# andrei-ace/EdgeStyle

Hardware: AMD Instinct MI355X
Metric: 512x512 try-on images/sec @ 50 DDIM steps (6-cond ControlNet) (higher is better)
Workload: dtype f16; 1 GPU; BASELINE configs[1]: full 6-cond edgestyle_multicontrolnet + controllora, 512x512, 50 DDIM steps, CFG 7.5, batch=1/GPU, hipGraph-captured step, cond embedding + VAE decode included; images_per_gpu=1, ddim_steps=50, parallelism=dp1 (independent images, one RCCL gather)

## Files before the change

### edgestyle_amd/csrc/builder.hip

```cpp
#include <hip/hip_runtime.h>
#include <math.h>
#include <stdio.h>
#include <stdlib.h>
#include <string.h>

#include <algorithm>
#include <deque>
#include <functional>
#include <map>
#include <memory>
#include <stdexcept>
#include <string>
#include <thread>
#include <unordered_map>
#include <vector>

#include "../../include/edgestyle_hip.h"
#include "plan.h"

extern "C" void es_set_error(const char* msg);
extern "C" int es_plan_set_dry(int on);

namespace {

// ... 335 lines not shown
bool groups_tile_256(const es_launch_query& q) {
  for (int g = 0; g < std::min(q.n_counts, 4); ++g) if ((q.group_n[g] * q.hw) % 256) return false;
  return true;
}
bool launch_takes_xs(const es_launch_query& q, const es_launch_knobs& k) {
  const bool xs_res = !q.has_residual || (k.xs_residual && q.kpad == 320 && !q.geglu && !q.has_ln && q.residual_dense && !(q.wide && wide_stream(q.dtype, k)));
  if (!(q.ksize == 1 && q.stride == 1 && !q.upsample && !q.C2 && !q.has_temb && xs_res && !q.n_tails && q.x_rep == 1 && q.act == ES_ACT_NONE &&
        q.unit_scale && !q.force_splitk && !k.force_bn && k.xs_enabled)) return false;
  if (q.ngroups > 1 && (q.ngroups > 4 || !groups_tile_256(q) || !q.groups_agree)) return false;
  return xs_shape_ok(q.M, q.ksize, q.kpad, q.cin, q.ctail, q.cout, q.geglu != 0, k.xs_min_m);
}
bool launch_choose(const es_launch_query& q, const es_launch_knobs& k, es_launch_choice* o) {
  memset(o, 0, sizeof(*o));
  if (launch_takes_xs(q, k)) { o->route = ES_ROUTE_LINEAR_XS; return true; }
  const bool aligned = q.C1 % BK == 0 && q.C2 % BK == 0;
  const bool big_ok = k.big_tile && aligned && !q.geglu && !q.has_ln && groups_tile_256(q);
  const bool small_ok = k.small_tile && aligned && !q.geglu && k.force_waves != 8;
  const bool ln256_ok = k.big_tile_256 && (q.geglu || q.has_ln) && q.ksize == 1 && q.stride == 1 && !q.upsample && !q.C2 && !q.n_tails && !q.has_temb &&
                        q.x_rep == 1 && q.C1 % BK == 0 && q.rows_padded % 256 == 0 && q.cout % 8 == 0 && !(q.geglu && q.has_residual) && !q.wide &&
                        q.gn_groups == 0 && k.force_waves != 8 && groups_tile_256(q);
  int cand[5], nc = 0;
  if (ln256_ok) cand[nc++] = 256;
  if (big_ok) cand[nc++] = 320;
  cand[nc++] = 160; cand[nc++] = 128;
  if (small_ok) cand[nc++] = 64;
  if (k.force_bn) { cand[0] = k.force_bn; nc = 1; }
  const bool geglu = q.geglu != 0, allow_split = !q.has_ln;
  int bn, splitk, stages;
  if (!plan_gemm(q.M, q.rows_padded, q.kpad, geglu, cand, nc, allow_split, &bn, &splitk, &stages)) return false;
  if (bn == 320 && !k.force_bn && (q.force_splitk ? q.force_splitk : splitk) == 1 &&
      !es_conv_gemm8p_form_ok(geglu ? ES_ACT_GEGLU : q.act, q.cout, q.has_temb, q.hw, q.has_residual)) {
    const int at = (int)(std::find(cand, cand + nc, 320) - cand);
    std::copy(cand + at + 1, cand + nc, cand + at);
    if (!plan_gemm(q.M, q.rows_padded, q.kpad, geglu, cand, nc - 1, allow_split, &bn, &splitk, &stages)) return false;
  }
  if (stages == 4 && !k.deep_ring) stages = 2;
  if (q.force_splitk) { splitk = q.force_splitk; stages = q.stages; }
  else if (q.stages) stages = q.stages;
  if (!stages) stages = k.force_stages;
  o->bn = bn; o->splitk = splitk; o->stages = stages;
  if (k.force_waves) o->waves = k.force_waves;
  else if (k.eight_waves && q.ksize == 1 && q.M <= 65536 && aligned && bn != 64 && bn != 320 && bn != 256 && !(stages == 4 && bn != 128) && stages != 3) o->waves = 8;
  o->xcd_m_fastest = k.xcd_order < 0 ? (q.ngroups <= 1 && splitk == 1 && q.M <= 2048 && q.w_numel > q.src_numel) : k.xcd_order;
  const int cstore = geglu ? q.cout / 2 : q.cout;
  o->gn_partials = q.gn_groups > 0 && gn_handover(q.hw, cstore, q.gn_groups, k) && !geglu && !q.has_ln && q.cout / q.gn_groups <= (bn == 320 ? 160 : bn);
  o->wide = q.wide && q.has_residual && wide_stream(q.dtype, k) && cstore % 8 == 0 && !geglu;
  return true;
}
bool launch_gn_fold(const es_launch_query& q, int groups, const es_launch_knobs& k) {
  if (!(k.gn_fold && k.xs_enabled) || k.gn_handover || q.hw % 256 || groups < 1 || groups > 32) return false;
  if (q.geglu || q.has_ln || q.kpad % groups || !xs_shape_fits(q.ksize, q.kpad, q.cin, q.ctail, q.cout, false)) return false;
  if (q.M < (q.kpad == 320 ? 8192 : 32768)) return false;
  return !(q.ngroups > 1 && (q.ngroups > 4 || !groups_tile_256(q) || !q.groups_agree));
}
struct BuildEnv { es_launch_knobs knobs; bool chunk_major; };
BuildEnv read_build_env() {
  auto env = [](const char* name, const char* dflt) { const char* e = getenv(name); return std::string(e ? e : dflt); };
  const std::string ho = env("ES_GN_HANDOVER", "0"), ws = env("ES_WIDE_STREAM", "auto");
  BuildEnv b;
  b.chunk_major = env("ES_CHUNK_MAJOR", "0") == "1";
  es_launch_knobs& k = b.knobs;
  memset(&k, 0, sizeof(k));
  k.xs_enabled = k.big_tile = k.small_tile = k.eight_waves = k.deep_ring = 1; k.xs_min_m = XS_MIN_M; k.xcd_order = -1;
  k.xs_residual = env("ES_XS_RESIDUAL", "1") == "1"; k.big_tile_256 = env("ES_BIG_TILE_256", "1")[0] != '0'; k.gn_fold = env("ES_GN_FOLD", "1") == "1";
  k.gn_handover = ho == "all" ? 2 : ho == "1"; k.wide_stream = ws == "auto" ? -1 : ws == "1";
  return b;
}

struct Builder {
  Heap heap;
  unsigned long long ws_bytes = 0;
  int dt = ES_F16;
  const BuildEnv env = read_build_env();
  std::vector<std::pair<unsigned long long, std::vector<char>>> uploads;
  std::deque<PW> pws;
  std::map<std::string, const PW*> pack_cache;
  std::map<const void*, unsigned long long> vec_cache;
  std::map<std::pair<int, int>, unsigned long long> gn_partials, fusion_scratch;
  std::map<int, unsigned long long> zero_bias;

  T empty(int n, int h, int w, int c, int es = 2) {
    T t; t.n = n; t.h = h; t.w = w; t.c = c; t.ld = c; t.es = es;
    auto blk = std::make_shared<Blk>();
    blk->heap = &heap; blk->bytes = std::max<size_t>(t.bytes(), 1); blk->off = heap.alloc(blk->bytes);
    t.b = blk; t.p = FAKE_HEAP + blk->off;
    return t;
  }
  unsigned long long persistent(size_t bytes) { return FAKE_HEAP + heap.alloc(std::max<size_t>(bytes, 1)); }
  T persistent_t(int n, int h, int w, int c, int es = 2) {
    T t; t.n = n; t.h = h; t.w = w; t.c = c; t.ld = c; t.es = es;
    t.p = persistent(t.bytes());
    return t;
  }
  char* staged(unsigned long long addr, size_t bytes) {
    uploads.emplace_back(addr, std::vector<char>(bytes, 0));
    return uploads.back().second.data();
  }
  unsigned long long upload_f32(const std::vector<float>& v) {
    const unsigned long long a = persistent(v.size() * 4);
    memcpy(staged(a, v.size() * 4), v.data(), v.size() * 4);
    return a;
  }
  unsigned long long workspace(unsigned long long bytes) { ws_bytes = std::max(ws_bytes, bytes); return FAKE_WS; }
  void add_into(const T& a, const T& b, const T& out) {
    if (!a.contig() || !b.contig() || !out.contig() || a.numel() != b.numel() || a.numel() != out.numel()) fail("builder: add of non-contiguous or differently sized tensors");
    ok(es_add(a.ptr(), b.ptr(), out.ptr(), a.numel(), dt, nullptr), "es_add");
// ... 313 lines not shown
    return out;
  }

  T group_norm(const T& x, const std::vector<Norm>& nl, int groups, float eps, bool silu, const T& x2 = T(), const std::vector<int>& group_n = {}) {
    const int N = x.n, C1 = x.c, C2 = x2 ? x2.c : 0;
    T out = empty(N, x.h, x.w, C1 + C2);
    auto key = std::make_pair(N, groups);
    auto it = gn_partials.find(key);
    if (it == gn_partials.end()) it = gn_partials.emplace(key, persistent(es_group_norm_partials_bytes(N, groups))).first;
    es_gn_desc d;
    memset(&d, 0, sizeof(d));
    d.x = x.ptr(); d.x2 = x2 ? x2.ptr() : nullptr; d.out = out.ptr(); d.partials = (float*)it->second;
    if (nl.size() > 1) {
      int sum = 0;
      for (int n : group_n) sum += n;
      if (nl.size() > 4 || group_n.size() != nl.size() || sum != N) fail("grouped group_norm: bad group table");
      d.ngroups = (int)nl.size();
      int acc = 0;
      for (size_t g = 0; g < nl.size(); ++g) { acc += group_n[g]; d.n_end[g] = acc; d.gamma_g[g] = (const float*)nl[g].g; d.beta_g[g] = (const float*)nl[g].b; }
    } else { d.gamma = (const float*)nl[0].g; d.beta = (const float*)nl[0].b; }
    d.N = N; d.HW = (int)x.hw(); d.C1 = C1; d.C2 = C2; d.groups = groups; d.eps = eps; d.silu = silu; d.dtype = dt;
    if (x.gnp && !x2 && gn_handover(x.hw(), C1, groups, env.knobs) && x.gnp_groups == groups) {
      d.partials = (float*)x.gnp; d.ext_chunks = (int)(2 * (x.hw() / 64));
    }
    ok(es_group_norm(&d, nullptr), "es_group_norm");
    return out;
  }
  T group_norm(const T& x, const Norm& n, int groups, float eps, bool silu, const T& x2 = T()) { return group_norm(x, std::vector<Norm>{n}, groups, eps, silu, x2); }

  T gn_proj_in(const T& x, const std::vector<Norm>& nl, int groups, float eps, const PWs& pl, const std::vector<int>& group_n = {}) {
    const int N = x.n;
    const long long hw = x.hw(), M = (long long)N * hw;
    const bool grouped = pl.size() > 1;
    CA g; g.group_n = group_n;
    es_launch_query q = launch_query(pl, M, hw, g, x.c, 0, x.numel(), false);
    for (const PW* p : pl)
      if (p->rows_padded != pl[0]->rows_padded || p->kpad != pl[0]->kpad || p->cout != pl[0]->cout || p->geglu != pl[0]->geglu) q.groups_agree = 0;
    if (!(x.contig() && launch_gn_fold(q, groups, env.knobs))) return conv_gemm(group_norm(x, nl, groups, eps, false, T(), group_n), pl, g);
    auto key = std::make_pair(N, groups);
    auto it = gn_partials.find(key);
    if (it == gn_partials.end()) it = gn_partials.emplace(key, persistent(es_group_norm_partials_bytes(N, groups))).first;
    es_gn_desc d;
    memset(&d, 0, sizeof(d));
    d.x = x.ptr(); d.partials = (float*)it->second;
    d.N = N; d.HW = (int)hw; d.C1 = x.c; d.C2 = 0; d.groups = groups; d.eps = eps; d.silu = 0; d.dtype = dt; d.stats_only = 1;
    ok(es_group_norm(&d, nullptr), "es_group_norm");
    T out = empty(N, x.h, x.w, pl[0]->cout);
    GnFront gn;
    gn.part = it->second; gn.nl = nl; gn.groups = groups; gn.nchunk = es_group_norm_chunks((int)hw); gn.hw = (int)hw; gn.eps = eps;
    std::vector<long long> rows;
    if (grouped) for (int n : group_n) rows.push_back(n * hw);
    linear_xs(x.view((int)M, 1, 1, x.c), pl, M, out.view((int)M, 1, 1, pl[0]->cout), rows, T(), &gn);
    return out;
  }

  T timestep_embedding(const T& t, int n, int dim) {
    T out = empty(n, 1, 1, dim);
    ok(es_timestep_embedding((const float*)t.ptr(), out.ptr(), n, dim, dt, nullptr), "es_timestep_embedding");
    return out;
  }
  void memcpy_t(const T& dst, const T& src) {
    if (!dst.contig() || !src.contig() || dst.bytes() != src.bytes()) fail("memcpy: contiguous tensors of equal byte size");
    ok(es_memcpy(dst.ptr(), src.ptr(), src.bytes(), nullptr), "es_memcpy");
  }
  void memcpy2d(unsigned long long dst, size_t dpitch, unsigned long long src, size_t spitch, size_t width, size_t height) {
    ok(es_memcpy2d((void*)dst, dpitch, (const void*)src, spitch, width, height, nullptr), "es_memcpy2d");
  }
  void gather_row(const T& table, int nrows, const T& idx, const T& out, int row_len) {
    ok(es_gather_row((const float*)table.ptr(), (const int32_t*)idx.ptr(), (float*)out.ptr(), row_len, nrows, nullptr), "es_gather_row");
  }
};

struct UCfg {
  int in_ch, out_ch, nb, ch[4], has_attn[4], lpb, heads, cross, groups; float eps;
  int nce, ce[4], cond_ch;
};
struct VCfg { int nb, ch[4], lpb, latent, groups; float eps, scaling; int scale() const { return 1 << (nb - 1); } };

struct Resnet {
  Norm n1, n2;
  const PW *conv1 = nullptr, *conv2 = nullptr, *shortc = nullptr, *conv2s = nullptr;
  int groups = 32; float eps = 1e-5f; int temb_off = -1;
  Resnet() {}
  Resnet(Builder& B, const Weights& W, const std::string& p, int groups_, float eps_, int temb_off_) : groups(groups_), eps(eps_), temb_off(temb_off_) {
    const es_tensor* w1 = W.get(p + ".conv1.weight");
    const int cin = (int)w1->shape[1], cout = (int)w1->shape[0];
    W.shaped(p + ".conv1.weight", {cout, cin, 3, 3}); W.shaped(p + ".conv2.weight", {cout, cout, 3, 3});
    if (W.has(p + ".conv_shortcut.weight")) W.shaped(p + ".conv_shortcut.weight", {cout, cin, 1, 1});
    else if (cin != cout) fail("es_load_weights: '" + p + "' changes the channel count but has no conv_shortcut");
    if (temb_off_ >= 0) W.shaped(p + ".time_emb_proj.weight", {cout, -1});
    n1 = B.norm(W, p + ".norm1", cin); n2 = B.norm(W, p + ".norm2", cout);
    conv1 = B.conv(W, p + ".conv1");
    const bool has_short = W.has(p + ".conv_shortcut.weight");
    if (has_short && cout % 64 == 0 && cin % 64 == 0) conv2s = B.conv_tail(W, p + ".conv2", p + ".conv_shortcut");
    else { conv2 = B.conv(W, p + ".conv2"); if (has_short) shortc = B.conv(W, p + ".conv_shortcut"); }
  }
  T run(Builder& B, const T& x, const T& tproj, const T& x2 = T()) const {
    T h = B.group_norm(x, n1, groups, eps, true, x2);
    CA a;
    if (temb_off >= 0) { a.temb = tproj.chan(temb_off, tproj.c - temb_off); a.temb_stride = tproj.ld; }
    a.gn_groups = groups;
    h = B.conv_gemm(h, conv1, a);
    h = B.group_norm(h, n2, groups, eps, true);
    if (conv2s) {
      if (x2 && (x.c % 64 || x2.c % 64)) fail("builder: skip concat with channels that are not multiples of 64");
      CA t; t.tails.push_back(x); if (x2) t.tails.push_back(x2); t.gn_groups = groups;
// ... 249 lines not shown
    }
    h = B.group_norm(h, d_norm, cfg.groups, cfg.eps, true);
    return B.conv_gemm(h, d_out);
  }
};

struct Model {
  Builder B;
  UCfg ucfg; VCfg vcfg;
  es_ctx_geometry geo;
  Dict d_unet, d_vae, d_fusion, d_cn[6];
  UNet unet;
  VAE vae;
  std::vector<std::unique_ptr<ControlNet>> nets;
  std::vector<int> net_of_cond;
  std::vector<std::pair<int, std::vector<int>>> groups;
  std::vector<FusionParams> fusion;
  std::vector<std::pair<int, int>> table;
  std::vector<const Encoder*> encs; std::vector<int> counts; int ntot = 0, width = 0, ncn = 0;
  int B_ = 1, N = 2, T_ = 50, h = 64, w = 64, nn = 6, kmax = 3;
  T latents, model_in, noise, ehs, step_idx, t_rows, scales_cur, t_table, scale_table, coef, ts_dev, image;
  std::vector<T> conds, cond_img, cond_noise, gbufs, hist;
  std::vector<T> ctx_grouped, ctx_unet; std::vector<std::vector<T>> ctx_nets;
  T cond_cat, tproj_table, tproj_cur, tproj_gen;
  std::vector<T> fused_zero, fz_zero, fz_u;
  bool guess = false;
  int Bc = 2;
  std::vector<std::vector<T>> ctx_guess;

  std::vector<Norm> norms(const std::vector<const Resnet*>& rs, int which) const { std::vector<Norm> v; for (auto r : rs) v.push_back(which == 1 ? r->n1 : r->n2); return v; }

  T g_resnet(const std::vector<const Resnet*>& rs, const T& x, const T& tproj) {
    const Resnet* r0 = rs[0];
    T hh = B.group_norm(x, norms(rs, 1), r0->groups, r0->eps, true, T(), counts);
    PWs c1, c2, c2s, sh; bool all_s = true;
    for (auto r : rs) { c1.push_back(r->conv1); c2.push_back(r->conv2); c2s.push_back(r->conv2s); sh.push_back(r->shortc); if (!r->conv2s) all_s = false; }
    CA a; a.temb = tproj.chan(r0->temb_off, tproj.c - r0->temb_off); a.temb_stride = tproj.ld; a.group_n = counts; a.gn_groups = r0->groups;
    hh = B.conv_gemm(hh, c1, a);
    hh = B.group_norm(hh, norms(rs, 2), r0->groups, r0->eps, true, T(), counts);
    if (all_s) { CA t; t.tails.push_back(x); t.group_n = counts; t.gn_groups = r0->groups; return B.conv_gemm(hh, c2s, t); }
    for (auto r : rs) if (r->conv2s) fail("builder: grouped resnets must fold conv_shortcut all alike");
    T xs = x;
    if (r0->shortc) { CA s; s.group_n = counts; xs = B.conv_gemm(x, sh, s); }
    CA r; r.residual = xs; r.group_n = counts; r.wide = true; r.gn_groups = r0->groups;
    return B.conv_gemm(hh, c2, r);
  }
  T g_transformer(const std::vector<const Transformer*>& ts, const T& x, const T& kv) {
    const Transformer* t0 = ts[0];
    const int Nn = x.n, H = x.h, Wd = x.w, C = x.c;
    std::vector<int> rows;
    for (int n : counts) rows.push_back(n * H * Wd);
    std::vector<Norm> nl; PWs pin, qkv, o1, q2, o2, ff1, ffo;
    for (auto t : ts) { nl.push_back(t->norm); pin.push_back(t->proj_in); qkv.push_back(t->qkv_ln); o1.push_back(t->o1); q2.push_back(t->q2_ln); o2.push_back(t->o2); ff1.push_back(t->ff1_ln); ffo.push_back(t->ffo); }
    T tok = B.gn_proj_in(x, nl, t0->groups, 1e-6f, pin, counts).view(Nn, H * Wd, 1, C);
    CA gr; gr.group_n = rows;
    T q = B.linear(tok, qkv, gr);
    T a = B.attention(q.chan(0, C), q.chan(C, C), q.chan(2 * C, C), t0->heads);
    CA r1 = gr; r1.residual = tok; r1.wide = true;
    tok = B.linear(a, o1, r1);
    T qq = B.linear(tok, q2, gr);
    a = B.attention(qq, kv.chan(0, C), kv.chan(C, C), t0->heads);
    CA r2 = gr; r2.residual = tok; r2.wide = true;
    tok = B.linear(a, o2, r2);
    T f = B.linear(tok, ff1, gr);
    CA fo; fo.x2 = tok.view(Nn, H, Wd, C); fo.residual = x; fo.group_n = counts; fo.wide = true; fo.gn_groups = t0->groups;
    return B.conv_gemm(f.view(Nn, H, Wd, 4 * C), ffo, fo);
  }
  void g_run(T hh, const T& tproj, std::vector<T>& skips, T& mid) {
    const Encoder* e0 = encs[0];
    skips.push_back(hh);
    int ci = 0;
    auto rs_of = [&](const std::function<const Resnet*(const Encoder*)>& f) { std::vector<const Resnet*> v; for (auto e : encs) v.push_back(f(e)); return v; };
    auto ts_of = [&](int ti) { std::vector<const Transformer*> v; for (auto e : encs) v.push_back(&e->tr[ti]); return v; };
    for (size_t i = 0; i < e0->down.size(); ++i) {
      for (size_t j = 0; j < e0->down[i].size(); ++j) {
        hh = g_resnet(rs_of([&](const Encoder* e) { return &e->down[i][j].first; }), hh, tproj);
        if (e0->down[i][j].second >= 0) { hh = g_transformer(ts_of(e0->down[i][j].second), hh, ctx_grouped[ci]); ++ci; }
        skips.push_back(hh);
      }
      if (e0->downsample[i]) {
        PWs ds; for (auto e : encs) ds.push_back(e->downsample[i]);
        CA a; a.stride = 2; a.group_n = counts; a.gn_groups = ucfg.groups;
        hh = B.conv_gemm(hh, ds, a);
        skips.push_back(hh);
      }
    }
    hh = g_resnet(rs_of([](const Encoder* e) { return &e->mid0; }), hh, tproj);
    hh = g_transformer(ts_of(e0->mid_attn), hh, ctx_grouped[ci]);
    mid = g_resnet(rs_of([](const Encoder* e) { return &e->mid1; }), hh, tproj);
  }
  T transformer(const Transformer& t, const T& x, const T& kv) {
    const int Nn = x.n, H = x.h, Wd = x.w, C = x.c;
    T tok = B.gn_proj_in(x, std::vector<Norm>{t.norm}, t.groups, 1e-6f, PWs{t.proj_in}).view(Nn, H * Wd, 1, C);
    T q = B.linear(tok, t.qkv_ln);
    T a = B.attention(q.chan(0, C), q.chan(C, C), q.chan(2 * C, C), t.heads);
    CA r1; r1.residual = tok; r1.wide = true;
    tok = B.linear(a, t.o1, r1);
    T qq = B.linear(tok, t.q2_ln);
    a = B.attention(qq, kv.chan(0, C), kv.chan(C, C), t.heads);
    CA r2; r2.residual = tok; r2.wide = true;
    tok = B.linear(a, t.o2, r2);
    T f = B.linear(tok, t.ff1_ln);
    CA fo; fo.x2 = tok.view(Nn, H, Wd, C); fo.residual = x; fo.wide = true; fo.gn_groups = t.groups;
    return B.conv_gemm(f.view(Nn, H, Wd, 4 * C), t.ffo, fo);
  }

  void set_context() {
    size_t gi = 0;
    for (const auto& g : groups) {
      const ControlNet& net = *nets[g.first];
      for (int ti = 0; ti < net.n_enc_tr; ++ti) net.tr[ti].context(B, ehs, ctx_nets[gi][ti], (int)g.second.size());
      ++gi;
    }
    for (size_t ti = 0; ti < unet.tr.size(); ++ti) unet.tr[ti].context(B, ehs, ctx_unet[ti], 1);
  }
  void set_conds() {
    int a = 0;
    for (const auto& g : groups) for (int p : g.second) { B.memcpy_t(cond_cat.batch(a, N), conds[p]); a += N; }
  }
  void set_time_table() {
    int a = 0;
    const size_t es = 2;
    for (size_t e = 0; e < encs.size(); ++e) {
      T proj = encs[e]->time_proj(B, ts_dev, T_);
      const size_t wb = (size_t)encs[e]->tproj_width() * es;
      for (int j = 0; j < counts[e]; ++j)
        B.memcpy2d(tproj_table.p + (unsigned long long)(a + j) * width * es, (size_t)ntot * width * es, proj.p, wb, wb, (size_t)T_);
      a += counts[e];
    }
  }
  T time_proj_generic() {
    const size_t es = 2;
    int a = 0;
    for (size_t e = 0; e < encs.size(); ++e) {
      T proj = encs[e]->time_proj(B, t_rows, counts[e]);
      const size_t wb = (size_t)encs[e]->tproj_width() * es;
      B.memcpy2d(tproj_gen.p + (unsigned long long)a * width * es, (size_t)width * es, proj.p, wb, wb, (size_t)counts[e]);
      a += counts[e];
    }
    return tproj_gen;
  }
  std::vector<T> fuse(const std::vector<std::vector<T>>& rpn, int Nf, const std::vector<T>* addends) {
    const size_t nl = rpn[0].size();
    std::vector<es_fusion_desc> fd(nl);
    std::vector<T> us, outs;
    for (size_t k = 0; k < nl; ++k) {
      const FusionParams& fp = fusion[k];
      const int HW = fp.s * fp.s, Cc = fp.c;
      auto key = std::make_pair(Nf, (int)k);
      auto it = B.fusion_scratch.find(key);
      if (it == B.fusion_scratch.end()) it = B.fusion_scratch.emplace(key, B.persistent(es_fusion_scratch_bytes(Nf))).first;
      T u = B.empty(Nf, HW, 1, Cc), out = B.empty(Nf, HW, 1, Cc);
      es_fusion_desc& d = fd[k];
      memset(&d, 0, sizeof(d));
      for (int i = 0; i < 6; ++i) { d.res[i] = rpn[i][k].ptr(); d.res_bs[i] = rpn[i][k].bstride(); d.res_scale[i] = 1.f; }
// ... 202 lines not shown
      }
    }
  }

  void pack_fusion(const Weights& W) {
    for (size_t i = 0; i < table.size(); ++i) {
      const std::string p = i + 1 < table.size() ? "multi_controlnet_down_blocks." + std::to_string(i) : "multi_controlnet_mid_block";
      const int c = table[i].first, s = table[i].second, hw = s * s;
      FusionParams f; f.c = c; f.s = s;
      f.w1 = B.upload_f32(to_f32(W.shaped(p + ".first_conv.weight", {3 * c, 2, 1, 1})));
      f.b1 = B.upload_f32(to_f32(W.shaped(p + ".first_conv.bias", {3 * c})));
      f.w2 = B.upload_f32(to_f32(W.shaped(p + ".second_conv.weight", {c, 3, 1, 1})));
      f.b2 = B.upload_f32(to_f32(W.shaped(p + ".second_conv.bias", {c})));
      f.w3 = B.upload_f32(to_f32(W.shaped(p + ".third_conv.weight", {c, 1, 1, 1})));
      f.b3 = B.upload_f32(to_f32(W.shaped(p + ".third_conv.bias", {c})));
      auto plane = [&](const std::string& key, int per) {
        const std::vector<float> t = to_f32(W.shaped(key, {(long long)per * c, s, s}));
        const unsigned long long a = B.persistent((size_t)hw * c * per * 2);
        uint16_t* d = (uint16_t*)B.staged(a, (size_t)hw * c * per * 2);
        parallel_for(hw, [&](long long x0, long long x1) {
          for (long long px = x0; px < x1; ++px)
            for (int cc = 0; cc < c * per; ++cc) d[(size_t)px * c * per + cc] = B.enc(t[(size_t)cc * hw + px]);
        });
        return a;
      };
      f.g1 = plane(p + ".first_normalization.weight", 3); f.be1 = plane(p + ".first_normalization.bias", 3);
      f.g2 = plane(p + ".second_normalization.weight", 1); f.be2 = plane(p + ".second_normalization.bias", 1);
      fusion.push_back(f);
    }
  }
};

struct Recording {
  es_plan* p;
  explicit Recording(es_plan* pl) : p(pl) { if (es_plan_begin_record(p)) fail(std::string("es_load_weights: ") + es_last_error()); es_plan_set_dry(1); }
  ~Recording() { es_plan_set_dry(0); es_plan_end_record(p); }
};

}

extern "C" int es_plan_gemm_choice(long long M, int rows_padded, int kpad, int geglu, const int* bns, int n_bns, int allow_split, int* bn, int* splitk, int* stages) {
  if (!bns || n_bns < 1 || !bn || !splitk || !stages) { es_set_error("es_plan_gemm_choice: null argument"); return -1; }
  if (!plan_gemm(M, rows_padded, kpad, geglu != 0, bns, n_bns, allow_split != 0, bn, splitk, stages)) { es_set_error("es_plan_gemm_choice: rows_padded fits no N tile"); return -1; }
  return 0;
}
extern "C" int es_linear_xs_eligible(long long M, int ksize, int kpad, int cin, int ctail, int cout, int geglu) {
  return xs_shape_ok(M, ksize, kpad, cin, ctail, cout, geglu != 0, XS_MIN_M) ? 1 : 0;
}
extern "C" int es_launch_choose(const es_launch_query* q, const es_launch_knobs* k, es_launch_choice* out) {
  if (!q || !k || !out) { es_set_error("es_launch_choose: null argument"); return -1; }
  if (!launch_choose(*q, *k, out)) { es_set_error("es_launch_choose: rows_padded fits no N tile"); return -1; }
  return 0;
}
extern "C" int es_launch_route(const es_launch_query* q, const es_launch_knobs* k) { return q && k && launch_takes_xs(*q, *k) ? ES_ROUTE_LINEAR_XS : ES_ROUTE_CONV_GEMM; }
extern "C" int es_launch_gn_fold(const es_launch_query* q, int groups, const es_launch_knobs* k) { return q && k && launch_gn_fold(*q, groups, *k); }
extern "C" int es_launch_gn_handover(long long hw, int c, int groups, const es_launch_knobs* k) { return k && gn_handover(hw, c, groups, *k); }
extern "C" int es_launch_wide_stream(int dtype, const es_launch_knobs* k) { return k && wide_stream(dtype, *k); }

extern "C" int es_load_weights(const es_weights* wts, const es_model_config* mc, const es_ctx_geometry* g, int device, es_ctx** out) {
  if (!wts || !mc || !g || !out) { es_set_error("es_load_weights: null argument"); return -1; }
  es_ctx* ctx = nullptr;
  es_plan* plans[ES_PLAN_COUNT] = {};
  void* arena = nullptr;
  try {
    auto m = std::make_unique<Model>();
    Model& M = *m;
    Builder& B = M.B;
    if (mc->n_blocks < 2 || mc->n_blocks > 4 || mc->vae_n_blocks < 2 || mc->vae_n_blocks > 4) fail("es_load_weights: 2..4 resolution levels");
    if (g->n_conds != 6 && g->n_conds != 1) fail("es_load_weights: n_conds is 6 (the reference's fused multi-ControlNet model, MC:66-114) or 1 (a single ControlNet, PL:338-351)");
    if (g->n_conds == 1 && wts->n_controlnets != 1) fail("es_load_weights: a single-ControlNet context takes exactly one ControlNet");
    if (g->dtype != ES_F16 && g->dtype != ES_BF16) fail("es_load_weights: dtype must be ES_F16 or ES_BF16");
    if (g->B < 1 || g->h < 1 || g->w < 1 || g->n_steps < 1) fail("es_load_weights: bad geometry");
    if (wts->n_controlnets < 1 || wts->n_controlnets > 6) fail("es_load_weights: 1..6 distinct ControlNets");
    UCfg& u = M.ucfg;
    u.in_ch = mc->in_channels; u.out_ch = mc->out_channels; u.nb = mc->n_blocks; u.lpb = mc->layers_per_block; u.heads = mc->num_heads;
    u.cross = mc->cross_attention_dim; u.groups = mc->norm_num_groups; u.eps = mc->norm_eps; u.nce = mc->n_cond_embed; u.cond_ch = mc->conditioning_channels;
    for (int i = 0; i < 4; ++i) { u.ch[i] = mc->block_out_channels[i]; u.has_attn[i] = mc->down_has_attn[i]; u.ce[i] = mc->cond_embed_channels[i]; }
    VCfg& v = M.vcfg;
    v.nb = mc->vae_n_blocks; v.lpb = mc->vae_layers_per_block; v.latent = mc->vae_latent_channels; v.groups = mc->vae_norm_num_groups;
    v.eps = mc->vae_norm_eps; v.scaling = mc->vae_scaling_factor;
    for (int i = 0; i < 4; ++i) v.ch[i] = mc->vae_block_out_channels[i];
    if (u.in_ch != v.latent) fail("es_load_weights: the UNet's in_channels must equal the VAE's latent_channels");
    if (u.cond_ch != 3 || u.nce < 2 || u.nce > 4) fail("es_load_weights: conditioning embedding of 3 input channels, 2..4 widths");
    M.geo = *g;
    B.dt = g->dtype;
    M.B_ = g->B; M.N = g->cfg ? 2 * g->B : g->B; M.T_ = g->n_steps; M.h = g->h; M.w = g->w; M.nn = g->n_conds;
    M.guess = g->guess_mode != 0;
    M.Bc = M.guess ? g->B : M.N;
    const int N = M.N, TS = M.T_, h = g->h, w = g->w, Bn = g->B, NN = g->n_conds, Nc = M.Bc;
    if (!M.guess) {
      int cnt[6] = {};
      for (int p = 0; p < NN; ++p) {
        const int ni = wts->net_of_cond[p];
        if (ni < 0 || ni >= wts->n_controlnets) fail("es_load_weights: net_of_cond names a ControlNet that was not given");
        ++cnt[ni];
      }
      const int hw_min = (h >> (u.nb - 1)) * (w >> (u.nb - 1));
      for (int i = 0; i <= wts->n_controlnets; ++i) {
        const long long n = (i < wts->n_controlnets ? (long long)cnt[i] : 1) * N;
        if (n && (n * hw_min) % BM) fail("es_load_weights: the groups of the lockstep pass do not tile in 128-pixel units at this latent size (the Python host falls back to serial chains; this builder does not)");
      }
    }
    M.d_unet.init(wts->unet, "UNet"); M.d_vae.init(wts->vae, "VAE"); M.d_fusion.init(wts->fusion, "fusion");
    for (int i = 0; i < wts->n_controlnets; ++i) M.d_cn[i].init(wts->controlnet[i], ("ControlNet " + std::to_string(i)).c_str());
    Weights Wu; Wu.own = &M.d_unet; Wu.who = "UNet";
    Weights Wv; Wv.own = &M.d_vae; Wv.who = "VAE";
// ... 202 lines not shown
```

### edgestyle_amd/csrc/elementwise.hip

```cpp
#include "common.h"
#include "../../include/edgestyle_hip.h"
#include "plan.h"
#include <string.h>

namespace {

thread_local char g_err[256] = "";

template <typename T>
__global__ void timestep_kernel(const float* __restrict__ t, T* __restrict__ out, int N, int dim) {
  const int half = dim / 2;
  const int i = blockIdx.x * blockDim.x + threadIdx.x;
  if (i >= N * half) return;
  const int n = i / half, k = i - n * half;
  const float f = expf(-9.210340371976184f * (float)k / (float)half);
  const float a = t[n] * f;
  out[(size_t)n * dim + k] = from_f32<T>(cosf(a));
  out[(size_t)n * dim + half + k] = from_f32<T>(sinf(a));
}

template <typename T>
__global__ void cfg_ddim_kernel(const T* __restrict__ noise, float* __restrict__ lat, T* __restrict__ model_in,
                                const float* __restrict__ coef, const int* __restrict__ step_idx, float gs, int B,
                                int HW, int L, int Ls, int cfg, int nsteps) {
// ... 282 lines not shown
  if (es_plan_recording()) { const es_op_incr a{ctr}; es_plan_record(ES_OP_INCR, &a, sizeof(a)); ES_PLAN_DRY_RETURN(); }
  hipLaunchKernelGGL(incr_kernel, dim3(1), dim3(1), 0, (hipStream_t)stream, ctr);
  ES_RET("es_incr");
}

extern "C" int es_gather_row(const float* table, const int32_t* idx, float* out, int row_len, int nrows,
                             void* stream) {
  if (!table || !idx || !out || row_len < 1 || nrows < 1) { es_set_error("es_gather_row: bad arguments"); return -1; }
  if (es_plan_recording()) { const es_op_gather_row a{table, idx, out, row_len, nrows}; es_plan_record(ES_OP_GATHER_ROW, &a, sizeof(a)); ES_PLAN_DRY_RETURN(); }
  hipLaunchKernelGGL(gather_row_kernel, dim3(nblk(row_len)), dim3(256), 0, (hipStream_t)stream, table, idx, out,
                     row_len, nrows);
  ES_RET("es_gather_row");
}

extern "C" int es_latents_to_input(const float* latents, void* model_in, int B, int HW, int L, int Lstride, int cfg,
                                   int dtype, void* stream) {
  if (!latents || !model_in || B < 1 || HW < 1 || L < 1 || Lstride < L) { es_set_error("es_latents_to_input: bad arguments"); return -1; }
  if (es_plan_recording()) { const es_op_latents_to_input a{latents, model_in, B, HW, L, Lstride, cfg, dtype}; es_plan_record(ES_OP_LATENTS_TO_INPUT, &a, sizeof(a)); ES_PLAN_DRY_RETURN(); }
  const long long n = (long long)B * HW * Lstride;
  if (dtype == ES_F16) hipLaunchKernelGGL(latents_to_input_kernel<f16>, dim3(nblk(n)), dim3(256), 0, (hipStream_t)stream, latents, (f16*)model_in, B, HW, L, Lstride, cfg);
  else hipLaunchKernelGGL(latents_to_input_kernel<bf16>, dim3(nblk(n)), dim3(256), 0, (hipStream_t)stream, latents, (bf16*)model_in, B, HW, L, Lstride, cfg);
  ES_RET("es_latents_to_input");
}

extern "C" int es_memcpy(void* dst, const void* src, size_t bytes, void* stream) {
  if (!dst || !src || !bytes) { es_set_error("es_memcpy: bad arguments"); return -1; }
  if (es_plan_recording()) { const es_op_memcpy a{dst, src, bytes}; es_plan_record(ES_OP_MEMCPY, &a, sizeof(a)); ES_PLAN_DRY_RETURN(); }
  if (hipMemcpyAsync(dst, src, bytes, hipMemcpyDeviceToDevice, (hipStream_t)stream) != hipSuccess) { es_set_error("es_memcpy: hipMemcpyAsync failed"); return -2; }
  return 0;
}

extern "C" int es_memcpy2d(void* dst, size_t dpitch, const void* src, size_t spitch, size_t width, size_t height, void* stream) {
  if (!dst || !src || !width || !height || dpitch < width || spitch < width) { es_set_error("es_memcpy2d: bad arguments"); return -1; }
  if (es_plan_recording()) { const es_op_memcpy2d a{dst, dpitch, src, spitch, width, height}; es_plan_record(ES_OP_MEMCPY2D, &a, sizeof(a)); ES_PLAN_DRY_RETURN(); }
  if (hipMemcpy2DAsync(dst, dpitch, src, spitch, width, height, hipMemcpyDeviceToDevice, (hipStream_t)stream) != hipSuccess) { es_set_error("es_memcpy2d: hipMemcpy2DAsync failed"); return -2; }
  return 0;
}

extern "C" int es_fill_f32(float* dst, float value, size_t n, void* stream) {
  if (!dst || !n) { es_set_error("es_fill_f32: bad arguments"); return -1; }
  if (es_plan_recording()) { const es_op_fill_f32 a{dst, n, value}; es_plan_record(ES_OP_FILL_F32, &a, sizeof(a)); ES_PLAN_DRY_RETURN(); }
  if (hipMemsetD32Async((hipDeviceptr_t)dst, __builtin_bit_cast(int, value), n, (hipStream_t)stream) != hipSuccess) { es_set_error("es_fill_f32: hipMemsetD32Async failed"); return -2; }
  return 0;
}

extern "C" size_t es_sizeof_desc(int which) {
  switch (which) {
    case 0: return sizeof(es_gemm_desc);
    case 1: return sizeof(es_attn_desc);
    case 2: return sizeof(es_gn_desc);
    case 3: return sizeof(es_fusion_desc);
    case 4: return sizeof(es_ln_desc);
    case 5: return sizeof(es_xs_desc);
    default: return 0;
  }
}
```

### edgestyle_amd/csrc/plan.h

```cpp
#pragma once
#include <stddef.h>
#include <stdint.h>

enum es_op_kind {
  ES_OP_CONV_GEMM = 1, ES_OP_LINEAR_XS, ES_OP_ATTENTION, ES_OP_GROUP_NORM, ES_OP_LAYER_NORM, ES_OP_LAYER_NORM_GROUPED,
  ES_OP_FUSION_BLOCK, ES_OP_FUSION_BLOCKS, ES_OP_TIMESTEP_EMBEDDING, ES_OP_CFG_DDIM, ES_OP_CFG_UNIPC, ES_OP_NCHW_TO_NHWC,
  ES_OP_NHWC_TO_NCHW, ES_OP_ADD, ES_OP_VAE_SAMPLE, ES_OP_INCR, ES_OP_GATHER_ROW, ES_OP_MEMCPY, ES_OP_MEMCPY2D,
  ES_OP_FILL_F32, ES_OP_LATENTS_TO_INPUT,
};

struct es_op_layer_norm { const void* x; void* out; const float* gamma; const float* beta; int M, C; float eps; int dtype; };
struct es_op_timestep { const float* t; void* out; int N, dim, dtype, pad_; };
struct es_op_cfg_ddim { const void* noise; float* latents; void* model_in; const float* coef; const int32_t* step_idx;
                        float guidance_scale; int B, HW, L, Lstride, cfg, nsteps, dtype; };
struct es_op_cfg_unipc { const void* noise; float* latents; float* last_sample; float* m0; float* m1; void* model_in;
                         const float* coef; const int32_t* step_idx; float guidance_scale; int B, HW, L, Lstride, cfg, nsteps, dtype; };
struct es_op_nchw_to_nhwc { const float* in; void* out; int N, C, HW, Cpad, dtype, pad_; };
struct es_op_nhwc_to_nchw { const void* in; float* out; int N, C, HW, Cstride; float scale, shift; int clamp01, dtype; };
struct es_op_add { const void* a; const void* b; void* y; int64_t n; int dtype, pad_; };
struct es_op_vae_sample { const void* moments; const float* noise; void* z; int N, HW, L, Lpad; float scaling; int dtype; };
struct es_op_incr { int32_t* ctr; };
struct es_op_gather_row { const float* table; const int32_t* idx; float* out; int row_len, nrows; };
struct es_op_memcpy { void* dst; const void* src; size_t bytes; };
struct es_op_memcpy2d { void* dst; size_t dpitch; const void* src; size_t spitch; size_t width, height; };
struct es_op_fill_f32 { float* dst; size_t n; float value; int pad_; };
struct es_op_latents_to_input { const float* latents; void* model_in; int B, HW, L, Lstride, cfg, dtype; };

extern "C" int es_plan_recording(void);
extern "C" void es_plan_record(int kind, const void* args, size_t bytes);
extern "C" int es_plan_dry(void);
#define ES_PLAN_RECORD(kind, ptr, bytes) do { if (es_plan_recording()) { es_plan_record((kind), (ptr), (bytes)); if (es_plan_dry()) return 0; } } while (0)
#define ES_PLAN_DRY_RETURN() do { if (es_plan_dry()) return 0; } while (0)

struct es_plan;
struct es_ctx;
int es_plan_relocate(es_plan* p, unsigned long long (*map)(unsigned long long addr, int use, void* user), void* user);
void es_ctx_adopt_arena(es_ctx* c, void* arena, size_t bytes, bool on_host);
void es_ctx_add_extent(es_ctx* c, unsigned long long off, unsigned long long bytes);

int es_image_resize_impl(const char* who, const es_image_u8* imgs, int count, uint8_t* out_u8, float* const* out_f32,
                         const int32_t* normalize, int R, void* workspace, size_t workspace_bytes, void* stream);

int es_randn_impl(const char* who, float* out, const es_randn_desc* d, void* stream, unsigned long long* advance);
```

### edgestyle_amd/csrc/plan.hip

```cpp
#include <hip/hip_runtime.h>
#include <dlfcn.h>
#include <math.h>
#include <stdio.h>
#include <stdlib.h>
#include <string.h>
#include <algorithm>
#include <string>
#include <utility>
#include <vector>

#include "../../include/edgestyle_hip.h"
#include "plan.h"

extern "C" void es_set_error(const char* msg);

struct es_plan {
  struct Op { int kind; size_t off, bytes; };
  std::vector<Op> ops;
  std::vector<char> blob;
};

namespace {
thread_local es_plan* g_rec = nullptr;
thread_local bool g_replaying = false;
thread_local bool g_dry = false;

struct RunOpts { const float* guidance = nullptr; const es_ctx* unipc = nullptr; };
int unipc_step(const es_ctx* c, const es_op_cfg_ddim* r, float guidance, void* s);

int launch_op(const es_plan* p, const es_plan::Op& op, hipStream_t st, const RunOpts& ro) {
  const float* guidance_override = ro.guidance;
  const char* a = p->blob.data() + op.off;
  void* s = (void*)st;
  switch (op.kind) {
    case ES_OP_CONV_GEMM: return es_conv_gemm((const es_gemm_desc*)a, s);
    case ES_OP_LINEAR_XS: return es_linear_xs((const es_xs_desc*)a, s);
    case ES_OP_ATTENTION: return es_attention((const es_attn_desc*)a, s);
    case ES_OP_GROUP_NORM: return es_group_norm((const es_gn_desc*)a, s);
    case ES_OP_LAYER_NORM: { auto* r = (const es_op_layer_norm*)a; return es_layer_norm(r->x, r->out, r->gamma, r->beta, r->M, r->C, r->eps, r->dtype, s); }
    case ES_OP_LAYER_NORM_GROUPED: return es_layer_norm_grouped((const es_ln_desc*)a, s);
    case ES_OP_FUSION_BLOCK: return es_fusion_block((const es_fusion_desc*)a, s);
    case ES_OP_FUSION_BLOCKS: return es_fusion_blocks((const es_fusion_desc*)a, (int)(op.bytes / sizeof(es_fusion_desc)), s);
    case ES_OP_TIMESTEP_EMBEDDING: { auto* r = (const es_op_timestep*)a; return es_timestep_embedding(r->t, r->out, r->N, r->dim, r->dtype, s); }
    case ES_OP_CFG_DDIM: { auto* r = (const es_op_cfg_ddim*)a;
      if (ro.unipc) return unipc_step(ro.unipc, r, guidance_override ? *guidance_override : r->guidance_scale, s);
      return es_cfg_ddim_step(r->noise, r->latents, r->model_in, r->coef, r->step_idx, guidance_override ? *guidance_override : r->guidance_scale,
                              r->B, r->HW, r->L, r->Lstride, r->cfg, r->nsteps, r->dtype, s); }
    case ES_OP_CFG_UNIPC: { auto* r = (const es_op_cfg_unipc*)a;
      return es_cfg_unipc_step(r->noise, r->latents, r->last_sample, r->m0, r->m1, r->model_in, r->coef, r->step_idx,
                               guidance_override ? *guidance_override : r->guidance_scale, r->B, r->HW, r->L, r->Lstride, r->cfg, r->nsteps, r->dtype, s); }
    case ES_OP_NCHW_TO_NHWC: { auto* r = (const es_op_nchw_to_nhwc*)a; return es_nchw_f32_to_nhwc(r->in, r->out, r->N, r->C, r->HW, r->Cpad, r->dtype, s); }
    case ES_OP_NHWC_TO_NCHW: { auto* r = (const es_op_nhwc_to_nchw*)a; return es_nhwc_to_nchw_f32(r->in, r->out, r->N, r->C, r->HW, r->Cstride, r->scale, r->shift, r->clamp01, r->dtype, s); }
    case ES_OP_ADD: { auto* r = (const es_op_add*)a; return es_add(r->a, r->b, r->y, r->n, r->dtype, s); }
    case ES_OP_VAE_SAMPLE: { auto* r = (const es_op_vae_sample*)a; return es_vae_sample(r->moments, r->noise, r->z, r->N, r->HW, r->L, r->Lpad, r->scaling, r->dtype, s); }
    case ES_OP_INCR: { auto* r = (const es_op_incr*)a; return es_incr(r->ctr, s); }
    case ES_OP_GATHER_ROW: { auto* r = (const es_op_gather_row*)a; return es_gather_row(r->table, r->idx, r->out, r->row_len, r->nrows, s); }
    case ES_OP_MEMCPY: { auto* r = (const es_op_memcpy*)a; return es_memcpy(r->dst, r->src, r->bytes, s); }
    case ES_OP_MEMCPY2D: { auto* r = (const es_op_memcpy2d*)a; return es_memcpy2d(r->dst, r->dpitch, r->src, r->spitch, r->width, r->height, s); }
    case ES_OP_FILL_F32: { auto* r = (const es_op_fill_f32*)a; return es_fill_f32(r->dst, r->value, r->n, s); }
    case ES_OP_LATENTS_TO_INPUT: { auto* r = (const es_op_latents_to_input*)a; return es_latents_to_input(r->latents, r->model_in, r->B, r->HW, r->L, r->Lstride, r->cfg, r->dtype, s); }
    default: es_set_error("es_plan_launch: unknown op"); return -1;
  }
}

int run_plan(const es_plan* p, hipStream_t st, const RunOpts& ro) {
  if (g_rec) { es_set_error("es_plan_launch: a plan is recording on this thread"); return -1; }
  g_replaying = true;
  int rc = 0;
  for (const auto& op : p->ops)
    if ((rc = launch_op(p, op, st, ro)) != 0) break;
  g_replaying = false;
  return rc;
}
}

extern "C" int es_plan_recording(void) { return g_rec != nullptr && !g_replaying; }
extern "C" void es_plan_record(int kind, const void* args, size_t bytes) {
  es_plan* p = g_rec;
  const size_t off = (p->blob.size() + 15) & ~(size_t)15;
  p->blob.resize(off + bytes);
  memcpy(p->blob.data() + off, args, bytes);
  p->ops.push_back({kind, off, bytes});
}

extern "C" int es_plan_dry(void) { return g_dry && g_rec != nullptr && !g_replaying; }
extern "C" int es_plan_set_dry(int on) { const int was = g_dry; g_dry = on != 0; return was; }
extern "C" es_plan* es_plan_create(void) { return new es_plan(); }
extern "C" void es_plan_destroy(es_plan* p) { if (g_rec == p) g_rec = nullptr; delete p; }
extern "C" int es_plan_begin_record(es_plan* p) {
  if (!p || g_rec) { es_set_error("es_plan_begin_record: null plan, or another plan is recording on this thread"); return -1; }
  g_rec = p;
  return 0;
}
extern "C" int es_plan_end_record(es_plan* p) {
  if (!p || g_rec != p) { es_set_error("es_plan_end_record: this plan is not recording"); return -1; }
  g_rec = nullptr;
  return 0;
}
extern "C" int es_plan_size(const es_plan* p) { return p ? (int)p->ops.size() : -1; }
extern "C" int es_plan_count(const es_plan* p, int kind) {
  if (!p) return -1;
  int n = 0;
  for (const auto& op : p->ops) n += op.kind == kind;
  return n;
}
extern "C" int es_plan_launch(const es_plan* p, void* stream) {
  if (!p) { es_set_error("es_plan_launch: null plan"); return -1; }
  return run_plan(p, (hipStream_t)stream, RunOpts{});
}

#include <stddef.h>
namespace {
struct PtrField { int off; int use; };
#define F_IN(S, m) {(int)offsetof(S, m), 1}
#define F_OUT(S, m) {(int)offsetof(S, m), 2}
#define F_IO(S, m) {(int)offsetof(S, m), 3}
#define F_IN4(S, m) {(int)offsetof(S, m), 1}, {(int)offsetof(S, m) + 8, 1}, {(int)offsetof(S, m) + 16, 1}, {(int)offsetof(S, m) + 24, 1}
const std::vector<PtrField>& ptr_fields(int kind, int& elem) {
  static const std::vector<PtrField> none;
  elem = 0;
  switch (kind) {
    case ES_OP_CONV_GEMM: { static const std::vector<PtrField> f = {
        F_IN(es_gemm_desc, x), F_IN(es_gemm_desc, x2), F_IN(es_gemm_desc, w), F_IN(es_gemm_desc, bias), F_IN(es_gemm_desc, temb),
        F_IN(es_gemm_desc, residual), F_IN(es_gemm_desc, out_scale_dev), F_OUT(es_gemm_desc, out), F_IO(es_gemm_desc, workspace),
        F_OUT(es_gemm_desc, prof), F_IN4(es_gemm_desc, w_g), F_IN4(es_gemm_desc, bias_g), F_IN(es_gemm_desc, ln_colsum),
        F_IN4(es_gemm_desc, ln_colsum_g), F_IN(es_gemm_desc, t1), F_IN(es_gemm_desc, t2), F_IN(es_gemm_desc, residual_lo),
        F_OUT(es_gemm_desc, out_lo), F_OUT(es_gemm_desc, gn_part)}; return f; }
    case ES_OP_LINEAR_XS: { static const std::vector<PtrField> f = {
        F_IN(es_xs_desc, x), F_OUT(es_xs_desc, out), F_IN(es_xs_desc, w), F_IN(es_xs_desc, bias), F_IN4(es_xs_desc, w_g),
        F_IN4(es_xs_desc, bias_g), F_OUT(es_xs_desc, prof), F_IN(es_xs_desc, residual), F_IN(es_xs_desc, gn_part), F_IN(es_xs_desc, gn_gamma),
        F_IN(es_xs_desc, gn_beta), F_IN4(es_xs_desc, gn_gamma_g), F_IN4(es_xs_desc, gn_beta_g)}; return f; }
    case ES_OP_ATTENTION: { static const std::vector<PtrField> f = {
        F_IN(es_attn_desc, q), F_IN(es_attn_desc, k), F_IN(es_attn_desc, v), F_OUT(es_attn_desc, o)}; return f; }
    case ES_OP_GROUP_NORM: { static const std::vector<PtrField> f = {
        F_IN(es_gn_desc, x), F_IN(es_gn_desc, x2), F_OUT(es_gn_desc, out), F_IN(es_gn_desc, gamma), F_IN(es_gn_desc, beta),
        F_IO(es_gn_desc, partials), F_IN4(es_gn_desc, gamma_g), F_IN4(es_gn_desc, beta_g)}; return f; }
    case ES_OP_LAYER_NORM: { static const std::vector<PtrField> f = {
        F_IN(es_op_layer_norm, x), F_OUT(es_op_layer_norm, out), F_IN(es_op_layer_norm, gamma), F_IN(es_op_layer_norm, beta)}; return f; }
    case ES_OP_LAYER_NORM_GROUPED: { static const std::vector<PtrField> f = {
        F_IN(es_ln_desc, x), F_OUT(es_ln_desc, out), F_IN4(es_ln_desc, gamma_g), F_IN4(es_ln_desc, beta_g)}; return f; }
    case ES_OP_FUSION_BLOCKS: elem = (int)sizeof(es_fusion_desc);
      [[fallthrough]];
    case ES_OP_FUSION_BLOCK: { static const std::vector<PtrField> f = {
        F_IN4(es_fusion_desc, res), {(int)offsetof(es_fusion_desc, res) + 32, 1}, {(int)offsetof(es_fusion_desc, res) + 40, 1},
        F_IN(es_fusion_desc, w1), F_IN(es_fusion_desc, b1), F_IN(es_fusion_desc, g1), F_IN(es_fusion_desc, be1),
        F_IN(es_fusion_desc, w2), F_IN(es_fusion_desc, b2), F_IN(es_fusion_desc, g2), F_IN(es_fusion_desc, be2),
        F_IN(es_fusion_desc, w3), F_IN(es_fusion_desc, b3), F_IO(es_fusion_desc, scratch), F_IO(es_fusion_desc, u),
        F_OUT(es_fusion_desc, out), F_IN(es_fusion_desc, res_scale_dev), F_IN(es_fusion_desc, addend)}; return f; }
    case ES_OP_TIMESTEP_EMBEDDING: { static const std::vector<PtrField> f = {F_IN(es_op_timestep, t), F_OUT(es_op_timestep, out)}; return f; }
    case ES_OP_CFG_DDIM: { static const std::vector<PtrField> f = {
        F_IN(es_op_cfg_ddim, noise), F_IO(es_op_cfg_ddim, latents), F_OUT(es_op_cfg_ddim, model_in), F_IN(es_op_cfg_ddim, coef),
        F_IN(es_op_cfg_ddim, step_idx)}; return f; }
    case ES_OP_CFG_UNIPC: { static const std::vector<PtrField> f = {
        F_IN(es_op_cfg_unipc, noise), F_IO(es_op_cfg_unipc, latents), F_IO(es_op_cfg_unipc, last_sample), F_IO(es_op_cfg_unipc, m0),
        F_IO(es_op_cfg_unipc, m1), F_OUT(es_op_cfg_unipc, model_in), F_IN(es_op_cfg_unipc, coef), F_IN(es_op_cfg_unipc, step_idx)}; return f; }
    case ES_OP_NCHW_TO_NHWC: { static const std::vector<PtrField> f = {F_IN(es_op_nchw_to_nhwc, in), F_OUT(es_op_nchw_to_nhwc, out)}; return f; }
    case ES_OP_NHWC_TO_NCHW: { static const std::vector<PtrField> f = {F_IN(es_op_nhwc_to_nchw, in), F_OUT(es_op_nhwc_to_nchw, out)}; return f; }
    case ES_OP_ADD: { static const std::vector<PtrField> f = {F_IN(es_op_add, a), F_IN(es_op_add, b), F_OUT(es_op_add, y)}; return f; }
    case ES_OP_VAE_SAMPLE: { static const std::vector<PtrField> f = {F_IN(es_op_vae_sample, moments), F_IN(es_op_vae_sample, noise), F_OUT(es_op_vae_sample, z)}; return f; }
    case ES_OP_INCR: { static const std::vector<PtrField> f = {F_IO(es_op_incr, ctr)}; return f; }
    case ES_OP_GATHER_ROW: { static const std::vector<PtrField> f = {F_IN(es_op_gather_row, table), F_IN(es_op_gather_row, idx), F_OUT(es_op_gather_row, out)}; return f; }
    case ES_OP_MEMCPY: { static const std::vector<PtrField> f = {F_OUT(es_op_memcpy, dst), F_IN(es_op_memcpy, src)}; return f; }
    case ES_OP_MEMCPY2D: { static const std::vector<PtrField> f = {F_OUT(es_op_memcpy2d, dst), F_IN(es_op_memcpy2d, src)}; return f; }
    case ES_OP_FILL_F32: { static const std::vector<PtrField> f = {F_OUT(es_op_fill_f32, dst)}; return f; }
    case ES_OP_LATENTS_TO_INPUT: { static const std::vector<PtrField> f = {F_IN(es_op_latents_to_input, latents), F_OUT(es_op_latents_to_input, model_in)}; return f; }
    default: return none;
  }
}
#undef F_IN
#undef F_OUT
#undef F_IO
#undef F_IN4
}
extern "C" int es_plan_pointer_fields(int kind, int32_t* offsets, int32_t* uses, int cap, int32_t* elem_bytes) {
  int elem = 0;
  const auto& f = ptr_fields(kind, elem);
  if (elem_bytes) *elem_bytes = elem;
  for (int i = 0; i < (int)f.size() && i < cap; ++i) {
    if (offsets) offsets[i] = f[i].off;
    if (uses) uses[i] = f[i].use;
  }
  return (int)f.size();
}

// ... 806 lines not shown
```

### edgestyle_amd/engine.py

```python
import os
import weakref
from typing import Dict, List, Optional, Sequence, Tuple

import torch

from . import lib as L
from . import ops
from .config import UNetConfig, VAEConfig

SD = Dict[str, torch.Tensor]


def fold_lora(sd: SD) -> SD:
    out = {k: v for k, v in sd.items() if ".lora_layer." not in k}
    for k in sd:
        if k.endswith(".lora_layer.down.weight"):
            base = k[: -len(".lora_layer.down.weight")]
            up = sd[base + ".lora_layer.up.weight"].double()
            out[base + ".weight"] = (sd[base + ".weight"].double() + up @ sd[k].double()).float()
    return out


_PACK_CACHE = {}

# ... 56 lines not shown
        self.conv1, self.conv2 = pk.conv(p + ".conv1"), pk.conv(p + ".conv2")
        self.short = pk.conv(p + ".conv_shortcut") if (p + ".conv_shortcut.weight") in pk.sd else None
        self.groups, self.eps, self.temb_off = groups, eps, temb_off
        self.cout = self.conv1.cout
        self.conv2s = None
        w2, ws_ = pk.sd[p + ".conv2.weight"], pk.sd.get(p + ".conv_shortcut.weight")
        if SHORTCUT_FOLD and ws_ is not None and w2.shape[1] % 64 == 0 and ws_.shape[1] % 64 == 0:
            self.conv2s = pk.conv_tail(p + ".conv2", p + ".conv_shortcut")

    def __call__(self, x, tproj, x2=None):
        h = ops.group_norm(x, self.n1[0], self.n1[1], self.groups, self.eps, True, x2=x2)
        temb = None if self.temb_off is None else tproj[:, self.temb_off:]
        h = ops.conv_gemm(h, self.conv1, temb=temb, gn_groups=self.groups)
        h = ops.group_norm(h, self.n2[0], self.n2[1], self.groups, self.eps, True)
        if self.conv2s is not None and (x2 is None or (x.shape[3] % 64 == 0 and x2.shape[3] % 64 == 0)):
            return ops.conv_gemm(h, self.conv2s, tail=(x, x2), gn_groups=self.groups)
        xs = ops.conv_gemm(x, self.short, x2=x2) if self.short is not None else x
        return ops.conv_gemm(h, self.conv2, residual=xs, wide=True, gn_groups=self.groups)


class Transformer:

    def __init__(self, pk: _Packer, p: str, heads: int, groups: int):
        tb = p + ".transformer_blocks.0"
        self.norm = pk.norm(p + ".norm")
        self.proj_in, self.proj_out = pk.conv(p + ".proj_in"), pk.conv(p + ".proj_out")
        self.ln1, self.ln2, self.ln3 = pk.norm(tb + ".norm1"), pk.norm(tb + ".norm2"), pk.norm(tb + ".norm3")
        self.qkv = pk.cat([tb + ".attn1.to_q", tb + ".attn1.to_k", tb + ".attn1.to_v"], bias=False)
        self.o1 = pk.conv(tb + ".attn1.to_out.0")
        self.q2 = pk.conv(tb + ".attn2.to_q")
        self.kv2 = pk.cat([tb + ".attn2.to_k", tb + ".attn2.to_v"], bias=False)
        self.o2 = pk.conv(tb + ".attn2.to_out.0")
        self.ff1 = pk.conv(tb + ".ff.net.0.proj", geglu=True)
        self.ff2 = pk.conv(tb + ".ff.net.2")
        self.heads, self.groups = heads, groups
        self.c = self.proj_in.cout
        self.ffo = None
        if FFO_FOLD and self.c % 64 == 0:
            wp = pk.t(p + ".proj_out.weight").reshape(self.c, self.c).double()
            wf, bf = pk.t(tb + ".ff.net.2.weight").double(), pk.t(tb + ".ff.net.2.bias").double()
            self.ffo = ops.pack_weight(torch.cat([wp @ wf, wp], 1).float(), (wp @ bf + pk.t(p + ".proj_out.bias").double()).float(),
                                       pk.dtype, pk.device)
        self.ln_fold = LN_FOLD and self.c % 64 == 0
        if self.ln_fold:
            self.qkv_ln = pk.cat_ln([tb + ".attn1.to_q", tb + ".attn1.to_k", tb + ".attn1.to_v"], False, tb + ".norm1")
            self.q2_ln = pk.cat_ln([tb + ".attn2.to_q"], False, tb + ".norm2")
            self.ff1_ln = pk.cat_ln([tb + ".ff.net.0.proj"], True, tb + ".norm3", geglu=True) if LN_FOLD_FF else None

    def context(self, ehs, out=None, rep: int = 1):
        return ops.linear(ehs, self.kv2, out=out, x_rep=rep)

    def __call__(self, x, kv):
        N, H, W, C = x.shape
        tok = ops.gn_proj_in(x, self.norm[0], self.norm[1], self.groups, 1e-6, self.proj_in).reshape(N, H * W, C)
        fold = self.ln_fold
        qkv = ops.linear(tok, self.qkv_ln) if fold else ops.linear(ops.layer_norm(tok, *self.ln1), self.qkv)
        a = ops.attention(qkv[:, :, :C], qkv[:, :, C:2 * C], qkv[:, :, 2 * C:], self.heads)
        tok = ops.linear(a, self.o1, residual=tok, wide=True)
        q = ops.linear(tok, self.q2_ln) if fold else ops.linear(ops.layer_norm(tok, *self.ln2), self.q2)
        a = ops.attention(q, kv[:, :, :C], kv[:, :, C:], self.heads)
        tok = ops.linear(a, self.o2, residual=tok, wide=True)
        f = ops.linear(tok, self.ff1_ln) if (fold and self.ff1_ln is not None) else ops.linear(ops.layer_norm(tok, *self.ln3), self.ff1)
        if self.ffo is not None:
            return ops.conv_gemm(f.reshape(N, H, W, 4 * C), self.ffo, x2=tok.reshape(N, H, W, C), residual=x, wide=True, gn_groups=self.groups)
        tok = ops.linear(f, self.ff2, residual=tok, wide=True)
        return ops.conv_gemm(tok.reshape(N, H, W, C), self.proj_out, residual=x, wide=True, gn_groups=self.groups)


class Encoder:

    def __init__(self, sd: SD, cfg: UNetConfig, dtype, device, extra_resnets: Sequence[str] = ()):
        sd = fold_lora(sd)
        self.cfg, self.dtype, self.device = cfg, dtype, device
        pk = self.pk = _Packer(sd, dtype, device)
        g, eps, heads = cfg.norm_num_groups, cfg.norm_eps, cfg.num_heads
        self.in_pad = (cfg.in_channels + 7) // 8 * 8
        self.conv_in = pk.conv("conv_in", cin_pad=self.in_pad)
        self.t1, self.t2 = pk.conv("time_embedding.linear_1"), pk.conv("time_embedding.linear_2")
        names = []
        ch = cfg.block_out_channels
        for i in range(len(ch)):
            for j in range(cfg.layers_per_block):
                names.append(f"down_blocks.{i}.resnets.{j}")
        names += ["mid_block.resnets.0", "mid_block.resnets.1"] + list(extra_resnets)
        offs, o = {}, 0
        for nme in names:
            offs[nme] = o
            o += sd[nme + ".time_emb_proj.weight"].shape[0]
        self.tproj = pk.cat([n + ".time_emb_proj" for n in names], bias=True)
        self.temb_offs = offs
        self.down: List[List[Tuple[Resnet, Optional[Transformer]]]] = []
        self.downsample: List[Optional[ops.PackedWeight]] = []
        for i in range(len(ch)):
            blk = []
            for j in range(cfg.layers_per_block):
                r = Resnet(pk, f"down_blocks.{i}.resnets.{j}", g, eps, offs[f"down_blocks.{i}.resnets.{j}"])
                a = Transformer(pk, f"down_blocks.{i}.attentions.{j}", heads, g) if cfg.down_has_attn[i] else None
                blk.append((r, a))
            self.down.append(blk)
            self.downsample.append(pk.conv(f"down_blocks.{i}.downsamplers.0.conv") if i != len(ch) - 1 else None)
        self.mid0 = Resnet(pk, "mid_block.resnets.0", g, eps, offs["mid_block.resnets.0"])
        self.mid_attn = Transformer(pk, "mid_block.attentions.0", heads, g)
        self.mid1 = Resnet(pk, "mid_block.resnets.1", g, eps, offs["mid_block.resnets.1"])

    def transformers(self) -> List[Transformer]:
        out = [a for blk in self.down for (_, a) in blk if a is not None]
        return out + [self.mid_attn]

    def context(self, ehs, outs: Optional[List[torch.Tensor]] = None) -> List[torch.Tensor]:
        tr = self.transformers()
        if outs is not None and outs[0].shape[0] == ehs.shape[0]:
            return [t.context(ehs, o) for t, o in zip(tr, outs)]
        return [t.context(ehs) for t in tr]

    def time_proj(self, t_dev: torch.Tensor, step_idx: Optional[torch.Tensor] = None) -> torch.Tensor:
# ... 213 lines not shown
        h = ops.conv_gemm(h, self.d_in)
        h = self._mid(self.d_mid, h)
        for rs, us in self.d_up:
            for r in rs:
                h = r(h, None)
            if us is not None:
                h = ops.conv_gemm(h, us, upsample=True)
        h = ops.group_norm(h, self.d_norm[0], self.d_norm[1], cfg.norm_num_groups, cfg.norm_eps, True)
        return ops.conv_gemm(h, self.d_out)


class GroupedEncoder:

    def __init__(self, encoders: Sequence[Encoder], counts: Sequence[int]):
        self.encs, self.counts = list(encoders), list(counts)
        e0 = self.encs[0]
        self.cfg = e0.cfg
        for e in self.encs[1:]:
            if e.cfg.block_out_channels != e0.cfg.block_out_channels or e.cfg.layers_per_block != e0.cfg.layers_per_block:
                raise L.EdgeStyleHipError("grouped encoders must share the architecture")
        self.ntot = sum(self.counts)
        self.width = max(e.tproj_width for e in self.encs)

    def groupable(self, hw_min: int) -> bool:
        return len(self.encs) <= 4 and all((n * hw_min) % ops.BM == 0 for n in self.counts)

    def time_proj(self, t_rows: torch.Tensor, out: Optional[torch.Tensor] = None) -> torch.Tensor:
        if out is None:
            out = torch.zeros((self.ntot, self.width), dtype=self.encs[0].dtype, device=t_rows.device)
        es = out.element_size()
        a = 0
        for e, n in zip(self.encs, self.counts):
            proj = e.time_proj(t_rows[:n])
            ops.memcpy2d(out[a].data_ptr(), self.width * es, proj.data_ptr(), e.tproj_width * es, e.tproj_width * es, n)
            a += n
        return out

    def _resnet(self, rs, x, tproj):
        c = self.counts
        r0 = rs[0]
        h = ops.group_norm(x, [r.n1[0] for r in rs], [r.n1[1] for r in rs], r0.groups, r0.eps, True, group_n=c)
        h = ops.conv_gemm(h, [r.conv1 for r in rs], temb=tproj[:, r0.temb_off:], group_n=c, gn_groups=r0.groups)
        h = ops.group_norm(h, [r.n2[0] for r in rs], [r.n2[1] for r in rs], r0.groups, r0.eps, True, group_n=c)
        if all(r.conv2s is not None for r in rs):
            return ops.conv_gemm(h, [r.conv2s for r in rs], tail=(x,), group_n=c, gn_groups=r0.groups)
        xs = ops.conv_gemm(x, [r.short for r in rs], group_n=c) if r0.short is not None else x
        return ops.conv_gemm(h, [r.conv2 for r in rs], residual=xs, group_n=c, wide=True, gn_groups=r0.groups)

    def _transformer(self, ts, x, kv):
        c = self.counts
        t0 = ts[0]
        N, H, W, C = x.shape
        rows = [n * H * W for n in c]
        tok = ops.gn_proj_in(x, [t.norm[0] for t in ts], [t.norm[1] for t in ts], t0.groups, 1e-6, [t.proj_in for t in ts], group_n=c).reshape(N, H * W, C)
        fold = all(t.ln_fold for t in ts)

        def ln_linear(k, plain, folded):
            if fold and folded is not None:
                return ops.linear(tok, [getattr(t, folded) for t in ts], group_n=rows)
            n = ops.layer_norm(tok, [getattr(t, k)[0] for t in ts], [getattr(t, k)[1] for t in ts], group_rows=rows)
            return ops.linear(n, [getattr(t, plain) for t in ts], group_n=rows)
        qkv = ln_linear("ln1", "qkv", "qkv_ln")
        a = ops.attention(qkv[:, :, :C], qkv[:, :, C:2 * C], qkv[:, :, 2 * C:], t0.heads)
        tok = ops.linear(a, [t.o1 for t in ts], residual=tok, group_n=rows, wide=True)
        q = ln_linear("ln2", "q2", "q2_ln")
        a = ops.attention(q, kv[:, :, :C], kv[:, :, C:], t0.heads)
        tok = ops.linear(a, [t.o2 for t in ts], residual=tok, group_n=rows, wide=True)
        f = ln_linear("ln3", "ff1", "ff1_ln" if all(t.ln_fold and t.ff1_ln is not None for t in ts) else None)
        if all(t.ffo is not None for t in ts):
            return ops.conv_gemm(f.reshape(N, H, W, 4 * C), [t.ffo for t in ts], x2=tok.reshape(N, H, W, C), residual=x, group_n=c, wide=True,
                                 gn_groups=t0.groups)
        tok = ops.linear(f, [t.ff2 for t in ts], residual=tok, group_n=rows, wide=True)
        return ops.conv_gemm(tok.reshape(N, H, W, C), [t.proj_out for t in ts], residual=x, group_n=c, wide=True, gn_groups=t0.groups)

    def run(self, h, tproj, ctx: List[torch.Tensor]):
        skips = [h]
        ci = 0
        e0 = self.encs[0]
        for i, blk in enumerate(e0.down):
            for j, (r, a) in enumerate(blk):
                h = self._resnet([e.down[i][j][0] for e in self.encs], h, tproj)
                if a is not None:
                    h = self._transformer([e.down[i][j][1] for e in self.encs], h, ctx[ci]); ci += 1
                skips.append(h)
            if e0.downsample[i] is not None:
                h = ops.conv_gemm(h, [e.downsample[i] for e in self.encs], stride=2, group_n=self.counts, gn_groups=e0.cfg.norm_num_groups)
                skips.append(h)
        h = self._resnet([e.mid0 for e in self.encs], h, tproj)
        h = self._transformer([e.mid_attn for e in self.encs], h, ctx[ci])
        h = self._resnet([e.mid1 for e in self.encs], h, tproj)
        return skips, h
```

### edgestyle_amd/lib.py

```python
import ctypes as C
import os

_HERE = os.path.dirname(os.path.abspath(__file__))
LIB_PATH = os.environ.get("ES_HIP_LIB") or os.path.join(_HERE, "lib", "libedgestyle_hip.so")

ES_F16, ES_BF16, ES_F32 = 0, 1, 2
ABI_VERSION = 7
ACT_NONE, ACT_SILU, ACT_GEGLU = 0, 1, 2


class GemmDesc(C.Structure):
    _fields_ = [
        ("x", C.c_void_p), ("x2", C.c_void_p), ("w", C.c_void_p), ("bias", C.c_void_p), ("temb", C.c_void_p),
        ("residual", C.c_void_p), ("out_scale_dev", C.c_void_p), ("out", C.c_void_p), ("workspace", C.c_void_p),
        ("prof", C.c_void_p),
        ("N", C.c_int32), ("Hsrc", C.c_int32), ("Wsrc", C.c_int32), ("C1", C.c_int32), ("C2", C.c_int32),
        ("Hout", C.c_int32), ("Wout", C.c_int32), ("Cout", C.c_int32),
        ("rows_padded", C.c_int32), ("Kpad", C.c_int32),
        ("ksize", C.c_int32), ("stride", C.c_int32), ("pad", C.c_int32),
        ("upsample", C.c_int32), ("temb_stride", C.c_int32), ("act", C.c_int32), ("splitk", C.c_int32),
        ("bn", C.c_int32), ("dtype", C.c_int32),
        ("ngroups", C.c_int32), ("mt_end", C.c_int32 * 4), ("w_g", C.c_void_p * 4), ("bias_g", C.c_void_p * 4),
        ("stages", C.c_int32), ("xcd_m_fastest", C.c_int32), ("waves", C.c_int32),
        ("out_scale", C.c_float),
        ("ln_colsum", C.c_void_p), ("ln_colsum_g", C.c_void_p * 4), ("ln_eps", C.c_float),
        ("t1", C.c_void_p), ("t2", C.c_void_p), ("Ct1", C.c_int32), ("Ct2", C.c_int32),
        ("x_nmod", C.c_int32), ("korder", C.c_int32), ("residual_lo", C.c_void_p), ("out_lo", C.c_void_p),
        ("gn_part", C.c_void_p), ("gn_groups", C.c_int32),
    ]


class XsDesc(C.Structure):
    _fields_ = [
        ("x", C.c_void_p), ("out", C.c_void_p), ("w", C.c_void_p), ("bias", C.c_void_p),
        ("w_g", C.c_void_p * 4), ("bias_g", C.c_void_p * 4), ("prof", C.c_void_p),
        ("mt_end", C.c_int32 * 4), ("ngroups", C.c_int32),
        ("M", C.c_int32), ("K", C.c_int32), ("Cout", C.c_int32), ("rows_padded", C.c_int32),
        ("ldo", C.c_int32), ("geglu", C.c_int32), ("ln", C.c_int32), ("ln_eps", C.c_float),
        ("nslices", C.c_int32), ("chunks_per_slice", C.c_int32), ("dtype", C.c_int32),
        ("residual", C.c_void_p),
        ("gn_part", C.c_void_p), ("gn_gamma", C.c_void_p), ("gn_beta", C.c_void_p), ("gn_gamma_g", C.c_void_p * 4), ("gn_beta_g", C.c_void_p * 4),
        ("gn_groups", C.c_int32), ("gn_nchunk", C.c_int32), ("gn_hw", C.c_int32), ("gn_eps", C.c_float),
    ]


class CtxGeometry(C.Structure):
    _fields_ = [("B", C.c_int32), ("cfg", C.c_int32), ("h", C.c_int32), ("w", C.c_int32),
                ("latent_channels", C.c_int32), ("latent_pad", C.c_int32), ("n_conds", C.c_int32),
                ("n_steps", C.c_int32), ("dtype", C.c_int32), ("guess_mode", C.c_int32)]


PLAN_STEP_GENERIC, PLAN_PREP, PLAN_STEP, PLAN_DECODE, PLAN_CONDS, PLAN_STEP_UNET = 0, 1, 2, 3, 4, 5
PLAN_COUNT = 6
(BUF_SAMPLE, BUF_T_ROWS, BUF_EHS, BUF_COND0, BUF_COND1, BUF_COND2, BUF_COND3, BUF_COND4, BUF_COND5, BUF_SCALES, BUF_NOISE,
 BUF_LATENTS, BUF_STEP_IDX, BUF_T_TABLE, BUF_SCALE_TABLE, BUF_COEF, BUF_TIMESTEPS, BUF_IMAGE) = range(18)
BUF_COND_IMG0, BUF_COND_NOISE0 = 18, 24
BUF_HIST0, BUF_COUNT = 30, 33
SCHED_DDIM, SCHED_UNIPC = 0, 1
OP_CONV_GEMM, OP_LINEAR_XS, OP_ATTENTION = 1, 2, 3


class AttnDesc(C.Structure):
    _fields_ = [
        ("q", C.c_void_p), ("k", C.c_void_p), ("v", C.c_void_p), ("o", C.c_void_p),
        ("N", C.c_int32), ("heads", C.c_int32), ("Sq", C.c_int32), ("Skv", C.c_int32), ("d", C.c_int32),
        ("ldq", C.c_int32), ("ldk", C.c_int32), ("ldv", C.c_int32), ("ldo", C.c_int32),
        ("bsq", C.c_int64), ("bsk", C.c_int64), ("bsv", C.c_int64), ("bso", C.c_int64),
        ("scale", C.c_float), ("dtype", C.c_int32),
    ]


class GnDesc(C.Structure):
    _fields_ = [
        ("x", C.c_void_p), ("x2", C.c_void_p), ("out", C.c_void_p),
        ("gamma", C.c_void_p), ("beta", C.c_void_p), ("partials", C.c_void_p),
        ("N", C.c_int32), ("HW", C.c_int32), ("C1", C.c_int32), ("C2", C.c_int32), ("groups", C.c_int32),
        ("eps", C.c_float), ("silu", C.c_int32), ("dtype", C.c_int32),
        ("ngroups", C.c_int32), ("n_end", C.c_int32 * 4), ("gamma_g", C.c_void_p * 4), ("beta_g", C.c_void_p * 4),
        ("ext_chunks", C.c_int32), ("stats_only", C.c_int32),
    ]


class LnDesc(C.Structure):
    _fields_ = [
        ("x", C.c_void_p), ("out", C.c_void_p), ("gamma_g", C.c_void_p * 4), ("beta_g", C.c_void_p * 4),
        ("row_end", C.c_int32 * 4), ("ngroups", C.c_int32), ("M", C.c_int32), ("C", C.c_int32),
        ("eps", C.c_float), ("dtype", C.c_int32),
    ]


class FusionDesc(C.Structure):
    _fields_ = [
        ("res", C.c_void_p * 6), ("res_bs", C.c_int64 * 6),
        ("w1", C.c_void_p), ("b1", C.c_void_p), ("g1", C.c_void_p), ("be1", C.c_void_p),
        ("w2", C.c_void_p), ("b2", C.c_void_p), ("g2", C.c_void_p), ("be2", C.c_void_p),
        ("w3", C.c_void_p), ("b3", C.c_void_p),
        ("scratch", C.c_void_p), ("u", C.c_void_p), ("out", C.c_void_p),
        ("res_scale_dev", C.c_void_p), ("addend", C.c_void_p),
        ("res_scale", C.c_float * 6),
        ("N", C.c_int32), ("HW", C.c_int32), ("C", C.c_int32),
        ("eps", C.c_float), ("dtype", C.c_int32),
    ]


class ImageU8(C.Structure):
    _fields_ = [("data", C.c_void_p), ("height", C.c_int32), ("width", C.c_int32), ("channels", C.c_int32), ("row_stride", C.c_int64)]


class Philox(C.Structure):
    _fields_ = [("seed", C.c_uint64), ("offset", C.c_uint64)]


# ... 18 lines not shown
NET_CONTROLNET, NET_CONTROL_LORA_VAE, NET_CONTROL_LORA = 0, 1, 2


class Weights(C.Structure):
    _fields_ = [("unet", StateDict), ("vae", StateDict), ("fusion", StateDict), ("controlnet", StateDict * 6),
                ("controlnet_kind", C.c_int32 * 6), ("n_controlnets", C.c_int32), ("net_of_cond", C.c_int32 * 6)]


class ModelConfig(C.Structure):
    _fields_ = [("in_channels", C.c_int32), ("out_channels", C.c_int32),
                ("n_blocks", C.c_int32), ("block_out_channels", C.c_int32 * 4), ("down_has_attn", C.c_int32 * 4),
                ("layers_per_block", C.c_int32), ("num_heads", C.c_int32), ("cross_attention_dim", C.c_int32),
                ("norm_num_groups", C.c_int32), ("norm_eps", C.c_float),
                ("n_cond_embed", C.c_int32), ("cond_embed_channels", C.c_int32 * 4), ("conditioning_channels", C.c_int32),
                ("text_tokens", C.c_int32),
                ("vae_n_blocks", C.c_int32), ("vae_block_out_channels", C.c_int32 * 4), ("vae_layers_per_block", C.c_int32),
                ("vae_latent_channels", C.c_int32), ("vae_norm_num_groups", C.c_int32),
                ("vae_norm_eps", C.c_float), ("vae_scaling_factor", C.c_float)]


_I32 = C.c_int32


class LaunchQuery(C.Structure):
    _fields_ = [(n, C.c_longlong) for n in ("M", "hw", "w_numel", "src_numel")] + \
        [(n, _I32) for n in ("ksize", "stride", "upsample", "C1", "C2", "rows_padded", "kpad", "cin", "ctail", "cout", "geglu", "has_ln", "act",
                             "has_temb", "has_residual", "residual_dense", "unit_scale", "n_tails", "x_rep", "wide", "dtype", "gn_groups",
                             "ngroups", "n_counts")] + [("group_n", _I32 * 4)] + [(n, _I32) for n in ("groups_agree", "force_splitk", "stages")]


class LaunchKnobs(C.Structure):
    _fields_ = [(n, _I32) for n in ("xs_enabled", "xs_residual", "xs_min_m", "big_tile", "big_tile_256", "small_tile", "eight_waves", "deep_ring",
                                    "gn_handover", "wide_stream", "gn_fold", "force_bn", "force_waves", "force_stages", "xcd_order")]


class LaunchChoice(C.Structure):
    _fields_ = [(n, _I32) for n in ("route", "bn", "splitk", "stages", "waves", "xcd_m_fastest", "gn_partials", "wide")]


ROUTE_CONV_GEMM, ROUTE_LINEAR_XS = 0, 1
XS_FORM_KC_MASK, XS_FORM_GEGLU, XS_FORM_LN, XS_FORM_RES, XS_FORM_PP, XS_FORM_GN = 0xFF, 0x100, 0x200, 0x400, 0x800, 0x1000
GN_FORM_SLAB, GN_FORM_TWO_LAUNCHES = 1, 2
GN_ROUTE_FIELDS = ("form", "gpb", "slots", "cpt", "ppb", "nchunk", "ps", "lanes", "blocks", "ipt", "general", "lds")

_P, _I, _F, _L = C.c_void_p, C.c_int, C.c_float, C.c_int64
SYMBOLS = {
    "es_abi_version": (C.c_int, []),
    "es_set_operand_limit": (C.c_ulonglong, [C.c_ulonglong]),
    "es_last_error": (C.c_char_p, []),
    "es_sizeof_desc": (C.c_size_t, [_I]),
    "es_conv_gemm": (C.c_int, [C.POINTER(GemmDesc), _P]),
    "es_conv_gemm_workspace_bytes": (C.c_size_t, [C.POINTER(GemmDesc)]),
    "es_linear_xs": (C.c_int, [C.POINTER(XsDesc), _P]),
    "es_linear_xs_set_pp": (C.c_int, [_I]),
    "es_linear_xs_last_form": (C.c_int, []),
    "es_attention": (C.c_int, [C.POINTER(AttnDesc), _P]),
    "es_attention_set_kvres": (C.c_int, [_I]),
    "es_attention_last_kernel": (C.c_int, []),
    "es_group_norm": (C.c_int, [C.POINTER(GnDesc), _P]),
    "es_group_norm_partials_bytes": (C.c_size_t, [_I, _I]),
    "es_group_norm_is_slab": (C.c_int, [_I, _I, _I]),
    "es_group_norm_chunks": (C.c_int, [_I]),
    "es_group_norm_route": (C.c_int, [C.POINTER(GnDesc), C.POINTER(C.c_int32)]),
    "es_layer_norm_route": (C.c_int, [_I]),
    "es_layer_norm": (C.c_int, [_P, _P, _P, _P, _I, _I, _F, _I, _P]),
    "es_fusion_block": (C.c_int, [C.POINTER(FusionDesc), _P]),
    "es_fusion_scratch_bytes": (C.c_size_t, [_I]),
    "es_fusion_blocks": (C.c_int, [C.POINTER(FusionDesc), _I, _P]),
    "es_timestep_embedding": (C.c_int, [_P, _P, _I, _I, _I, _P]),
    "es_cfg_ddim_step": (C.c_int, [_P, _P, _P, _P, _P, _F, _I, _I, _I, _I, _I, _I, _I, _P]),
    "es_cfg_unipc_step": (C.c_int, [_P, _P, _P, _P, _P, _P, _P, _P, _F, _I, _I, _I, _I, _I, _I, _I, _P]),
    "es_nchw_f32_to_nhwc": (C.c_int, [_P, _P, _I, _I, _I, _I, _I, _P]),
    "es_nhwc_to_nchw_f32": (C.c_int, [_P, _P, _I, _I, _I, _I, _F, _F, _I, _I, _P]),
    "es_add": (C.c_int, [_P, _P, _P, _L, _I, _P]),
    "es_vae_sample": (C.c_int, [_P, _P, _P, _I, _I, _I, _I, _F, _I, _P]),
    "es_incr": (C.c_int, [_P, _P]),
    "es_clock_probe": (C.c_int, [_P, C.c_uint, _P]),
    "es_gather_row": (C.c_int, [_P, _P, _P, _I, _I, _P]),
    "es_layer_norm_grouped": (C.c_int, [C.POINTER(LnDesc), _P]),
    "es_latents_to_input": (C.c_int, [_P, _P, _I, _I, _I, _I, _I, _I, _P]),
    "es_memcpy": (C.c_int, [_P, _P, C.c_size_t, _P]),
    "es_memcpy2d": (C.c_int, [_P, C.c_size_t, _P, C.c_size_t, C.c_size_t, C.c_size_t, _P]),
    "es_fill_f32": (C.c_int, [_P, _F, C.c_size_t, _P]),
    "es_plan_create": (_P, []),
    "es_plan_destroy": (None, [_P]),
    "es_plan_begin_record": (C.c_int, [_P]),
    "es_plan_end_record": (C.c_int, [_P]),
    "es_plan_size": (C.c_int, [_P]),
    "es_plan_count": (C.c_int, [_P, _I]),
    "es_plan_launch": (C.c_int, [_P, _P]),
    "es_ctx_create": (C.c_int, [_I, C.POINTER(_P)]),
    "es_ctx_destroy": (None, [_P]),
    "es_ctx_set_geometry": (C.c_int, [_P, C.POINTER(CtxGeometry)]),
    "es_ctx_set_plan": (C.c_int, [_P, _I, _P]),
    "es_ctx_bind": (C.c_int, [_P, _I, _P, C.c_size_t]),
    "es_ctx_buffer": (_P, [_P, _I, C.POINTER(C.c_size_t)]),
    "es_ctx_arena_bytes": (C.c_size_t, [_P]),
    "es_ctx_set_options": (C.c_int, [_P, C.POINTER(C.c_float), _F, _F, _I]),
    "es_ctx_set_scheduler": (C.c_int, [_P, _I]),
    "es_ctx_set_alphas_cumprod_f64": (C.c_int, [_P, C.POINTER(C.c_double), _I]),
    "es_unipc_coef_table": (C.c_int, [C.POINTER(C.c_double), _I, C.POINTER(C.c_float), _I, C.POINTER(C.c_float)]),
    "es_ctx_set_alphas_cumprod": (C.c_int, [_P, C.POINTER(C.c_float), _I]),
    "es_ctx_plan_size": (C.c_int, [_P, _I]),
    "es_ctx_plan": (_P, [_P, _I]),
    "es_ctx_load": (C.c_int, [C.c_char_p, _I, C.POINTER(_P)]),
    "es_ctx_save": (C.c_int, [_P, C.c_char_p]),
# ... 17 lines not shown
    "es_launch_wide_stream": (C.c_int, [_I, C.POINTER(LaunchKnobs)]),
    "es_conv_gemm8p_form_ok": (C.c_int, [_I, _I, _I, C.c_longlong, _I]),
    "es_ctx_graph_hazard": (C.c_int, []),
    "es_plan_set_dry": (C.c_int, [_I]),
    "es_image_fit": (C.c_int, [_I, _I, _I, C.POINTER(C.c_int32)]),
    "es_image_resize_coeffs": (C.c_int, [_I, _I, C.POINTER(C.c_int32), C.POINTER(C.c_int32), C.POINTER(C.c_int32), _I]),
    "es_image_resize_workspace_bytes": (C.c_size_t, [C.POINTER(ImageU8), _I, _I]),
    "es_image_resize_u8": (C.c_int, [C.POINTER(ImageU8), _I, _P, _I, _P, C.c_size_t, _P]),
    "es_image_u8_to_f32": (C.c_int, [_P, _P, _I, _I, _I, _I, _P]),
    "es_image_f32_to_u8": (C.c_int, [_P, _P, _I, _I, _I, _P]),
    "es_prepare_conds_u8": (C.c_int, [_P, C.POINTER(ImageU8), C.POINTER(C.c_int32), C.POINTER(_P), _P, C.c_size_t, _P]),
    "es_vae_decode_u8": (C.c_int, [_P, _P, _P, _P]),
    "es_philox4x32_10": (C.c_int, [C.POINTER(C.c_uint32), C.POINTER(C.c_uint32), C.POINTER(C.c_uint32)]),
    "es_philox_block_cap": (C.c_int, [_I]),
    "es_philox_blocks": (C.c_int, [_L, _I]),
    "es_philox_advance": (_L, [_L, _I]),
    "es_randn": (C.c_int, [_P, C.POINTER(RandnDesc), _P]),
    "es_randn_host": (C.c_int, [_P, C.POINTER(RandnDesc)]),
    "es_ctx_draw_latents": (C.c_int, [_P, C.POINTER(Philox), _I, _F, _I, _P, _P]),
    "es_ctx_draw_cond_noise": (C.c_int, [_P, C.POINTER(Philox), _I, _P]),
    "es_attention_causal": (C.c_int, [C.POINTER(AttnDesc), _P]),
    "es_text_embed": (C.c_int, [_P, _P, _P, _P, _I, _I, _I, _I, _I, _P]),
    "es_text_encoder_create": (C.c_int, [C.POINTER(StateDict), C.POINTER(TextConfig), _I, _I, _I, C.POINTER(_P)]),
    "es_text_encoder_destroy": (None, [_P]),
    "es_text_encoder_arena_bytes": (C.c_size_t, [_P]),
    "es_text_encode": (C.c_int, [_P, _P, _I, _P, _P]),
}

_lib = None


FUSION_MAX_BATCH = 13


class EdgeStyleHipError(RuntimeError):
    pass


def load():
    global _lib
    if _lib is not None:
        return _lib
    if not os.path.exists(LIB_PATH):
        raise EdgeStyleHipError(
            f"{LIB_PATH} not found: build it with `python -c 'import __graft_entry__ as g; g.build()'` "
            "(hipcc --offload-arch=gfx950). There is no CPU fallback for the product path.")
    lib = C.CDLL(LIB_PATH)
    for name, (res, args) in SYMBOLS.items():
        fn = getattr(lib, name)
        fn.restype = res
        fn.argtypes = args
    if lib.es_abi_version() != ABI_VERSION:
        raise EdgeStyleHipError("libedgestyle_hip.so ABI version mismatch")
    for i, st in enumerate((GemmDesc, AttnDesc, GnDesc, FusionDesc, LnDesc, XsDesc)):
        if lib.es_sizeof_desc(i) != C.sizeof(st):
            raise EdgeStyleHipError(f"descriptor layout mismatch for {st.__name__}: C {lib.es_sizeof_desc(i)} "
                                    f"vs ctypes {C.sizeof(st)}")
    _lib = lib
    return lib


def check(rc: int, what: str = ""):
    if rc != 0:
        msg = load().es_last_error()
        raise EdgeStyleHipError(f"{what} failed (rc={rc}): {msg.decode() if msg else ''}")


def group_norm_route(N: int, HW: int, C1: int, C2: int, groups: int, stats_only: bool = False, ext_chunks: int = 0) -> dict:
    d = GnDesc()
    d.N, d.HW, d.C1, d.C2, d.groups, d.stats_only, d.ext_chunks = N, HW, C1, C2, groups, 1 if stats_only else 0, ext_chunks
    out = (C.c_int32 * len(GN_ROUTE_FIELDS))()
    check(load().es_group_norm_route(C.byref(d), out), "es_group_norm_route")
    return dict(zip(GN_ROUTE_FIELDS, out))
```

### edgestyle_amd/ops.py

```python
import ctypes as C
import math
import os as _os
from dataclasses import dataclass
from typing import Optional, Sequence

import torch

from . import lib as L

_DT = {torch.float16: L.ES_F16, torch.bfloat16: L.ES_BF16}
LANE = 0


class lane:

    def __init__(self, i: int):
        self.i = i

    def __enter__(self):
        global LANE
        self.prev, LANE = LANE, self.i

    def __exit__(self, *a):
        global LANE
        LANE = self.prev


XCD_ORDER = -1
DEEP_RING = _os.environ.get("ES_DEEP_RING", "1") == "1"
FORCE_BN = 0
FORCE_STAGES = 0
FORCE_WAVES = 0
EIGHT_WAVES = _os.environ.get("ES_EIGHT_WAVES", "1") == "1"
SMALL_TILE = _os.environ.get("ES_SMALL_TILE", "1") == "1"
PROFILE = None


class Profiler:

    def __init__(self, device, capacity: int = 8192, stamps: bool = True):
        self.slots = torch.empty((capacity, 2), dtype=torch.int64, device=device)
        self.meta = []
        self.stamps = stamps
        self.descs = []
        self.reset()

    def reset(self):
        self.slots[:, 0] = 1 << 62
        self.slots[:, 1] = 0

    def next(self, meta) -> int:
        i = len(self.meta)
        if i >= self.slots.shape[0]:
            raise L.EdgeStyleHipError("Profiler capacity exceeded")
        self.meta.append(meta)
        return self.slots[i].data_ptr() if self.stamps else 0

    def replay_gemms(self, only_ksize: int = 0):
        lib = L.load()
        for d in self.descs:
            if only_ksize and (isinstance(d, L.XsDesc) or int(d.ksize) != only_ksize):
                continue
            fn = lib.es_linear_xs if isinstance(d, L.XsDesc) else lib.es_conv_gemm
            L.check(fn(C.byref(d), _stream()), "GEMM replay")

    def results(self, first: int = 0):
        s = self.slots[first:len(self.meta)].cpu().tolist()
        return [(m, (e - b) * 1e-8) for m, (b, e) in zip(self.meta[first:], s) if e > 0]
BK = 64
BM = 128


def _stream():
    return C.c_void_p(torch.cuda.current_stream().cuda_stream)


def _ptr(t: Optional[torch.Tensor]):
    return None if t is None else C.c_void_p(t.data_ptr())


def _dt(t: torch.Tensor) -> int:
    try:
        return _DT[t.dtype]
    except KeyError:
        raise L.EdgeStyleHipError(f"unsupported dtype {t.dtype}: the HIP path computes in fp16 or bf16")


@dataclass
class PackedWeight:
    w: torch.Tensor
    bias: Optional[torch.Tensor]
    cout: int
    cin: int
    ksize: int
    bn: int
    geglu: bool = False
    ln_colsum: Optional[torch.Tensor] = None
    ln_eps: float = 1e-5
    ctail: int = 0
    korder: int = 0

    @property
    def rows_padded(self):
        return self.w.shape[0]

    @property
    def kpad(self):
        return self.w.shape[1]


def choose_bn(cout: int) -> int:
    return 160 if (cout % 160 == 0 and cout % 128 != 0) else 128


CHUNK_MAJOR = _os.environ.get("ES_CHUNK_MAJOR", "0") == "1"

# ... 293 lines not shown
    lps = -(-lines // want)
    nslices = -(-lines // lps)
    d = L.XsDesc()
    d.x, d.out = x.data_ptr(), out.data_ptr()

    def bias_of(q):
        if q.bias is not None:
            return q.bias.data_ptr()
        key = (x.device, q.rows_padded)
        z = _zero_bias.get(key)
        if z is None:
            z = _zero_bias[key] = torch.zeros(q.rows_padded, dtype=torch.float32, device=x.device)
        return z.data_ptr()
    d.w, d.bias = pw.w.data_ptr(), bias_of(pw)
    d.M, d.K, d.Cout, d.rows_padded = M, K, pw.cout, pw.rows_padded
    d.ldo = ldo
    d.geglu, d.ln, d.ln_eps = int(pw.geglu), int(pw.ln_colsum is not None), pw.ln_eps
    d.nslices, d.chunks_per_slice, d.dtype = nslices, lps * pline, _dt(x)
    d.residual = residual.data_ptr() if residual is not None else None
    if gn is not None:
        d.gn_part, d.gn_groups, d.gn_nchunk, d.gn_hw, d.gn_eps = gn["part"].data_ptr(), gn["groups"], gn["nchunk"], gn["hw"], gn["eps"]
        gam, bet = gn["gamma"], gn["beta"]
        if pws is not None:
            if len(gam) != len(pws) or len(bet) != len(pws):
                raise L.EdgeStyleHipError("grouped linear_xs: one GroupNorm parameter set per weight group")
            for g in range(len(pws)):
                d.gn_gamma_g[g], d.gn_beta_g[g] = gam[g].data_ptr(), bet[g].data_ptr()
        else:
            if isinstance(gam, (list, tuple)):
                gam, bet = gam[0], bet[0]
            d.gn_gamma, d.gn_beta = gam.data_ptr(), bet.data_ptr()
    if pws is not None:
        d.ngroups = len(pws)
        acc = 0
        for g, (q, n) in enumerate(zip(pws, group_rows)):
            if (q.rows_padded, q.kpad, q.cout, q.geglu) != (pw.rows_padded, pw.kpad, pw.cout, pw.geglu):
                raise L.EdgeStyleHipError("grouped linear_xs: weight geometry differs between groups")
            acc += n
            d.mt_end[g] = (acc + 127) // 128
            d.w_g[g] = q.w.data_ptr()
            d.bias_g[g] = bias_of(q)
    if PROFILE is not None:
        d.prof = PROFILE.next((2.0 * M * pw.cout * K, 1, (M, pw.cout, K, 1, 1, 0),
                               dict(N=M, H=1, W=1, C1=K, C2=0, cout=pw.cout, k=1, stride=1, pad=0, upsample=False,
                                    geglu=pw.geglu, splitk=1, Hout=1, Wout=1, residual=residual is not None, temb=False, bn=0, stages=3,
                                    group_n=list(group_rows) if pws is not None else None, ctail=0, kernel="linear_xs",
                                    algorithmic_bytes=_algorithmic_bytes(x, None, pw, pws, out, residual))))
        dd = L.XsDesc()
        C.memmove(C.byref(dd), C.byref(d), C.sizeof(L.XsDesc))
        dd.prof = None
        PROFILE.descs.append(dd)
    L.check(L.load().es_linear_xs(C.byref(d), _stream()), "es_linear_xs")
    return out


WIDE_STREAM = _os.environ.get("ES_WIDE_STREAM", "auto")


GN_HANDOVER = _os.environ.get("ES_GN_HANDOVER", "0") in ("1", "all")


def gn_handover(hw: int, c: int, groups: int) -> bool:
    return bool(L.load().es_launch_gn_handover(hw, c, groups, C.byref(launch_knobs())))


GN_HANDOVER_ALL = _os.environ.get("ES_GN_HANDOVER", "0") == "all"


def wide_stream(dtype) -> bool:
    return bool(L.load().es_launch_wide_stream(_DT.get(dtype, L.ES_F32), C.byref(launch_knobs())))


def carry_lo(dst: torch.Tensor, src: torch.Tensor, shape=None) -> torch.Tensor:
    lo = getattr(src, "_lo", None)
    if lo is not None:
        dst._lo = lo.reshape(dst.shape if shape is None else shape)
    return dst


def conv_gemm(x: torch.Tensor, pw: PackedWeight, *, stride: int = 1, pad: Optional[int] = None,
              upsample: bool = False, x2: Optional[torch.Tensor] = None, temb: Optional[torch.Tensor] = None,
              residual: Optional[torch.Tensor] = None, act: int = L.ACT_NONE, out_scale: float = 1.0,
              out_scale_dev: Optional[torch.Tensor] = None, out: Optional[torch.Tensor] = None,
              out_hw=None, splitk: Optional[int] = None, stages: int = 0,
              group_n: Optional[Sequence[int]] = None, tail: Optional[Sequence[torch.Tensor]] = None,
              x_rep: int = 1, wide: bool = False, out_lo: Optional[torch.Tensor] = None, gn_groups: int = 0,
              gn_part: Optional[torch.Tensor] = None):
    pws = None
    if isinstance(pw, (list, tuple)):
        pws = list(pw)
        pw = pws[0]
        if len(pws) == 1:
            pws = None
    N, H, W, C1 = x.shape
    nsrc = N
    if x_rep > 1:
        if x2 is not None or tail:
            raise L.EdgeStyleHipError("conv_gemm: x_rep needs a single source")
        N = N * x_rep
    C2 = 0 if x2 is None else x2.shape[3]
    if C1 + C2 != pw.cin:
        raise L.EdgeStyleHipError(f"conv_gemm: input channels {C1}+{C2} != packed {pw.cin}")
    tails = [t for t in (tail or ()) if t is not None]
    if sum(t.shape[3] for t in tails) != pw.ctail or len(tails) > 2:
        raise L.EdgeStyleHipError(f"conv_gemm: tail channels {[t.shape[3] for t in tails]} != packed {pw.ctail}")
    k = pw.ksize
# ... 269 lines not shown
        d.ngroups = len(gl)
        acc = 0
        for g, n in enumerate(group_n):
            acc += n
            d.n_end[g] = acc
            d.gamma_g[g] = gl[g].data_ptr()
            d.beta_g[g] = bl[g].data_ptr()
        d.partials = part.data_ptr()
    else:
        d.gamma, d.beta, d.partials = gl[0].data_ptr(), bl[0].data_ptr(), part.data_ptr()
    gnp = getattr(x, "_gnp", None)
    if gnp is not None and partials is None and x2 is None and gn_handover(H * W, C1, groups) and gnp[1] == groups \
            and tuple(gnp[0].shape) == (N, 2 * (H * W // 64), groups, 2):
        d.partials, d.ext_chunks = gnp[0].data_ptr(), 2 * (H * W // 64)
    d.N, d.HW, d.C1, d.C2, d.groups = N, H * W, C1, C2, groups
    d.eps, d.silu, d.dtype = eps, 1 if silu else 0, _dt(x)
    L.check(L.load().es_group_norm(C.byref(d), _stream()), "es_group_norm")
    _drop_riders(out)
    return out


GN_FOLD = _os.environ.get("ES_GN_FOLD", "1") == "1"


def gn_fold_ok(M: int, hw: int, groups: int, pw: "PackedWeight", pws, group_n) -> bool:
    q = launch_query(M, hw, pw, pws, group_n)
    if pws is not None:
        q.groups_agree = all((p.rows_padded, p.kpad, p.cout, p.geglu, p.ln_colsum is None) == (pw.rows_padded, pw.kpad, pw.cout, pw.geglu, True) for p in pws)
    return bool(L.load().es_launch_gn_fold(C.byref(q), groups, C.byref(launch_knobs())))


def gn_proj_in(x: torch.Tensor, gamma, beta, groups: int, eps: float, pw, group_n: Optional[Sequence[int]] = None) -> torch.Tensor:
    N, H, W, Cc, _ = _gn_operands("gn_proj_in", x, None, groups)
    pws = list(pw) if isinstance(pw, (list, tuple)) and len(pw) > 1 else None
    p0 = pw[0] if isinstance(pw, (list, tuple)) else pw
    gl, bl = _norm_params("gn_proj_in", gamma, beta, Cc, x, nsets=None if pws is None else len(pws))
    M, hw = N * H * W, H * W
    if not gn_fold_ok(M, hw, groups, p0, pws, group_n):
        kw = {} if group_n is None else dict(group_n=group_n)
        return conv_gemm(group_norm(x, gamma, beta, groups, eps, False, **kw), pw, **kw)
    part = _gn_partials_for("gn_proj_in", x, N, groups)
    d = L.GnDesc()
    d.x, d.partials = x.data_ptr(), part.data_ptr()
    d.N, d.HW, d.C1, d.C2, d.groups = N, hw, Cc, 0, groups
    d.eps, d.silu, d.dtype, d.stats_only = eps, 0, _dt(x), 1
    L.check(L.load().es_group_norm(C.byref(d), _stream()), "es_group_norm")
    out = torch.empty((N, H, W, p0.cout), dtype=x.dtype, device=x.device)
    linear_xs(x.reshape(M, Cc), pws if pws is not None else p0, M, out.reshape(M, p0.cout),
              None if pws is None else [n * hw for n in group_n],
              gn=dict(part=part, gamma=gl, beta=bl, groups=groups, nchunk=L.load().es_group_norm_chunks(hw), hw=hw, eps=eps))
    return out


def layer_norm(x: torch.Tensor, gamma, beta, eps: float = 1e-5, group_rows: Optional[Sequence[int]] = None,
               out: Optional[torch.Tensor] = None) -> torch.Tensor:
    if x.dim() < 1 or x.dtype not in (torch.float16, torch.bfloat16):
        raise L.EdgeStyleHipError(f"layer_norm: x must be an fp16 or bf16 [..., C] tensor, not {x.dtype} {tuple(x.shape)}")
    Cc = x.shape[-1]
    if not x.is_contiguous() or Cc < 8 or Cc % 8 or x.numel() < Cc:
        raise L.EdgeStyleHipError(f"layer_norm: x must be contiguous, not empty and C a multiple of 8 (got shape {tuple(x.shape)}, strides {x.stride()})")
    if x.device.type != "meta" and x.data_ptr() % 16:
        raise L.EdgeStyleHipError("layer_norm: x must start at a multiple of 16 bytes (16-byte vector loads)")
    M = x.numel() // Cc
    grouped = isinstance(gamma, (list, tuple)) and len(gamma) > 1
    if grouped and (len(gamma) > 4 or group_rows is None or len(group_rows) != len(gamma) or sum(group_rows) != M):
        raise L.EdgeStyleHipError("grouped layer_norm: bad group table")
    gl, bl = _norm_params("layer_norm", gamma, beta, Cc, x)
    if not L.load().es_layer_norm_route(Cc):
        raise L.EdgeStyleHipError(f"layer_norm: C = {Cc} > 4096 unsupported")
    out = _norm_out("layer_norm", x, tuple(x.shape), out)
    if grouped:
        d = L.LnDesc()
        d.x, d.out = x.data_ptr(), out.data_ptr()
        acc = 0
        for g, n in enumerate(group_rows):
            acc += n
            d.row_end[g] = acc
            d.gamma_g[g] = gl[g].data_ptr()
            d.beta_g[g] = bl[g].data_ptr()
        d.ngroups, d.M, d.C, d.eps, d.dtype = len(gl), M, Cc, eps, _dt(x)
        L.check(L.load().es_layer_norm_grouped(C.byref(d), _stream()), "es_layer_norm_grouped")
    else:
        L.check(L.load().es_layer_norm(_ptr(x), _ptr(out), _ptr(gl[0]), _ptr(bl[0]), M, Cc, eps, _dt(x), _stream()), "es_layer_norm")
    _drop_riders(out)
    return out


def timestep_embedding(t: torch.Tensor, dim: int, dtype) -> torch.Tensor:
    N = t.numel()
    out = torch.empty((N, dim), dtype=dtype, device=t.device)
    L.check(L.load().es_timestep_embedding(_ptr(t), _ptr(out), N, dim, _DT[dtype], _stream()), "es_timestep_embedding")
    return out


def add(a: torch.Tensor, b: torch.Tensor, out: Optional[torch.Tensor] = None) -> torch.Tensor:
    if out is None:
        out = torch.empty_like(a)
    L.check(L.load().es_add(_ptr(a), _ptr(b), _ptr(out), a.numel(), _dt(a), _stream()), "es_add")
    _drop_riders(out)
    return out


def _drop_riders(t: torch.Tensor):
    for name in ("_lo", "_gnp"):
        if hasattr(t, name):
            delattr(t, name)
# ... 327 lines not shown
```

### include/edgestyle_hip.h

```cpp
#ifndef EDGESTYLE_HIP_H
#define EDGESTYLE_HIP_H
#include <stddef.h>
#include <stdint.h>

#ifdef __cplusplus
extern "C" {
#endif

enum { ES_F16 = 0, ES_BF16 = 1, ES_F32 = 2  };
enum { ES_ACT_NONE = 0, ES_ACT_SILU = 1, ES_ACT_GEGLU = 2 };

#define ES_ABI_VERSION 7
int es_abi_version(void);
size_t es_sizeof_desc(int which);
const char* es_last_error(void);

typedef struct {
  const void* x;
  const void* x2;
  const void* w;
  const float* bias;
  const void* temb;
  const void* residual;
  const float* out_scale_dev;
// ... 10 lines not shown
  int32_t splitk;
  int32_t bn;
  int32_t dtype;
  int32_t ngroups;
  int32_t mt_end[4];
  const void* w_g[4];
  const float* bias_g[4];
  int32_t stages;
  int32_t xcd_m_fastest;
  int32_t waves;
  float out_scale;
  const float* ln_colsum;
  const float* ln_colsum_g[4];
  float ln_eps;
  const void* t1;
  const void* t2;
  int32_t Ct1, Ct2;
  int32_t x_nmod;
  int32_t korder;
  const void* residual_lo;
  void* out_lo;
  float* gn_part;
  int32_t gn_groups;
} es_gemm_desc;
int es_conv_gemm(const es_gemm_desc* d, void* stream);
unsigned long long es_set_operand_limit(unsigned long long bytes);
size_t es_conv_gemm_workspace_bytes(const es_gemm_desc* d);

typedef struct {
  const void* x; void* out;
  const void* w; const float* bias;
  const void* w_g[4]; const float* bias_g[4];
  unsigned long long* prof;
  int32_t mt_end[4];
  int32_t ngroups;
  int32_t M, K, Cout, rows_padded;
  int32_t ldo;
  int32_t geglu, ln;
  float ln_eps;
  int32_t nslices, chunks_per_slice;
  int32_t dtype;
  const void* residual;
  const float* gn_part;
  const float* gn_gamma; const float* gn_beta;
  const float* gn_gamma_g[4]; const float* gn_beta_g[4];
  int32_t gn_groups, gn_nchunk, gn_hw;
  float gn_eps;
} es_xs_desc;
int es_linear_xs(const es_xs_desc* d, void* stream);
int es_linear_xs_set_pp(int on);
enum { ES_XS_FORM_KC_MASK = 0xFF, ES_XS_FORM_GEGLU = 0x100, ES_XS_FORM_LN = 0x200, ES_XS_FORM_RES = 0x400, ES_XS_FORM_PP = 0x800,
       ES_XS_FORM_GN = 0x1000 };
int es_linear_xs_last_form(void);

typedef struct {
  const void* q; const void* k; const void* v; void* o;
  int32_t N, heads, Sq, Skv, d;
  int32_t ldq, ldk, ldv, ldo;
  int64_t bsq, bsk, bsv, bso;
  float scale;
  int32_t dtype;
} es_attn_desc;
int es_attention(const es_attn_desc* d, void* stream);
int es_attention_set_kvres(int on);
int es_attention_last_kernel(void);

typedef struct {
  const void* x; const void* x2; void* out;
  const float* gamma; const float* beta; float* partials;
  int32_t N, HW, C1, C2, groups;
  float eps;
  int32_t silu, dtype;
  int32_t ngroups;
  int32_t n_end[4];
  const float* gamma_g[4];
  const float* beta_g[4];
  int32_t ext_chunks;
  int32_t stats_only;
} es_gn_desc;
int es_group_norm(const es_gn_desc* d, void* stream);
size_t es_group_norm_partials_bytes(int N, int groups);
int es_group_norm_chunks(int HW);
int es_group_norm_is_slab(int HW, int C, int groups);
enum {
  ES_GN_ROUTE_FORM = 0,
  ES_GN_ROUTE_GPB = 1,
  ES_GN_ROUTE_SLOTS = 2,
  ES_GN_ROUTE_CPT = 3,
  ES_GN_ROUTE_PPB = 4,
  ES_GN_ROUTE_NCHUNK = 5,
  ES_GN_ROUTE_PS = 6,
  ES_GN_ROUTE_LANES = 7,
  ES_GN_ROUTE_BLOCKS = 8,
  ES_GN_ROUTE_IPT = 9,
  ES_GN_ROUTE_GENERAL = 10,
  ES_GN_ROUTE_LDS = 11,
  ES_GN_ROUTE_FIELDS = 12
};
enum { ES_GN_FORM_SLAB = 1, ES_GN_FORM_TWO_LAUNCHES = 2 };
int es_group_norm_route(const es_gn_desc* d, int32_t out[ES_GN_ROUTE_FIELDS]);

int es_layer_norm(const void* x, void* out, const float* gamma, const float* beta, int M, int C, float eps,
                  int dtype, void* stream);
typedef struct {
  const void* x; void* out;
  const float* gamma_g[4]; const float* beta_g[4];
// ... 130 lines not shown
} es_weights;
typedef struct {
  int32_t in_channels, out_channels;
  int32_t n_blocks, block_out_channels[4], down_has_attn[4];
  int32_t layers_per_block, num_heads, cross_attention_dim, norm_num_groups;
  float norm_eps;
  int32_t n_cond_embed, cond_embed_channels[4], conditioning_channels;
  int32_t text_tokens;
  int32_t vae_n_blocks, vae_block_out_channels[4], vae_layers_per_block, vae_latent_channels, vae_norm_num_groups;
  float vae_norm_eps, vae_scaling_factor;
} es_model_config;
int es_load_weights(const es_weights* w, const es_model_config* cfg, const es_ctx_geometry* g, int device, es_ctx** out);
int es_plan_gemm_choice(long long M, int rows_padded, int kpad, int geglu, const int* bns, int n_bns, int allow_split,
                        int* bn, int* splitk, int* stages);
int es_linear_xs_eligible(long long M, int ksize, int kpad, int cin, int ctail, int cout, int geglu);
typedef struct {
  long long M, hw;
  long long w_numel, src_numel;
  int32_t ksize, stride, upsample, C1, C2;
  int32_t rows_padded, kpad, cin, ctail, cout, geglu, has_ln;
  int32_t act;
  int32_t has_temb, has_residual;
  int32_t residual_dense;
  int32_t unit_scale;
  int32_t n_tails, x_rep, wide;
  int32_t dtype, gn_groups;
  int32_t ngroups;
  int32_t n_counts, group_n[4];
  int32_t groups_agree;
  int32_t force_splitk, stages;
} es_launch_query;
typedef struct {
  int32_t xs_enabled, xs_residual, xs_min_m;
  int32_t big_tile, big_tile_256, small_tile, eight_waves;
  int32_t deep_ring;
  int32_t gn_handover;
  int32_t wide_stream;
  int32_t gn_fold;
  int32_t force_bn, force_waves, force_stages;
  int32_t xcd_order;
} es_launch_knobs;
enum { ES_ROUTE_CONV_GEMM = 0, ES_ROUTE_LINEAR_XS = 1 };
typedef struct {
  int32_t route;
  int32_t bn, splitk, stages, waves, xcd_m_fastest;
  int32_t gn_partials;
  int32_t wide;
} es_launch_choice;
int es_launch_choose(const es_launch_query* q, const es_launch_knobs* k, es_launch_choice* out);
int es_launch_route(const es_launch_query* q, const es_launch_knobs* k);
int es_launch_gn_fold(const es_launch_query* q, int groups, const es_launch_knobs* k);
int es_launch_gn_handover(long long hw, int c, int groups, const es_launch_knobs* k);
int es_launch_wide_stream(int dtype, const es_launch_knobs* k);
int es_conv_gemm8p_form_ok(int act, int cout, int has_temb, long long out_hw, int has_residual);
int es_ctx_graph_hazard(void);
int es_plan_set_dry(int on);

int es_ctx_launch_plan(es_ctx* c, int which, const float* guidance_scale, void* stream);
int es_ddim_coef_table(const float* alphas_cumprod, int n_alphas, const float* timesteps, int n, float* out);
int es_denoise_step(es_ctx* c, const void* sample, float t, const void* ehs, const void* const* cond_embeds,
                    const float* scales, void* out_noise, void* stream);
int es_denoise_loop(es_ctx* c, float* latents_inout, const void* ehs, float guidance_scale, const float* timesteps,
                    int n_steps, void* stream);
int es_vae_decode(es_ctx* c, const float* latents, float* out_img, void* stream);
int es_prepare_conds(es_ctx* c, const float* const* images, const float* const* noise, void* stream);

typedef struct {
  const uint8_t* data;
  int32_t height, width;
  int32_t channels;
  int64_t row_stride;
} es_image_u8;
int es_image_fit(int height, int width, int R, int32_t out[4]);
int es_image_resize_coeffs(int in, int out, int32_t* xmin, int32_t* ntaps, int32_t* k, int cap);
size_t es_image_resize_workspace_bytes(const es_image_u8* imgs, int count, int R);
int es_image_resize_u8(const es_image_u8* imgs, int count, uint8_t* out, int R, void* workspace, size_t workspace_bytes, void* stream);
int es_image_u8_to_f32(const uint8_t* in, float* out_nchw, int count, int H, int W, int normalize, void* stream);
int es_image_f32_to_u8(const float* in_nchw, uint8_t* out_hwc, int B, int H, int W, void* stream);
int es_prepare_conds_u8(es_ctx* c, const es_image_u8* images, const int32_t* normalize, const float* const* noise,
                        void* workspace, size_t workspace_bytes, void* stream);
int es_vae_decode_u8(es_ctx* c, const float* latents, uint8_t* out_hwc, void* stream);

typedef struct { uint64_t seed, offset; } es_philox;
typedef struct {
  uint64_t seed;
  uint64_t offset;
  int64_t numel;
  int32_t blocks;
  float scale;
  int32_t round_dtype;
  int64_t N, C, HW, Cstride;
} es_randn_desc;
int es_philox4x32_10(const uint32_t ctr[4], const uint32_t key[2], uint32_t out[4]);
int es_philox_block_cap(int device);
int es_philox_blocks(int64_t numel, int block_cap);
int64_t es_philox_advance(int64_t numel, int blocks);
int es_randn(float* out, const es_randn_desc* d, void* stream);
int es_randn_host(float* out, const es_randn_desc* d);
int es_ctx_draw_latents(es_ctx* c, es_philox* gens, int n_gens, float sigma, int round_dtype, float* latents_out, void* stream);
int es_ctx_draw_cond_noise(es_ctx* c, es_philox* gen, int round_dtype, void* stream);

int es_attention_causal(const es_attn_desc* d, void* stream);
int es_text_embed(const int32_t* ids, const float* tok, const float* pos, void* out, int rows, int S, int hidden, int vocab, int dtype,
                  void* stream);
typedef struct {
  int32_t vocab_size, hidden, heads, layers, intermediate, max_positions;
// ... 14 lines not shown
```

Measured before the change: 2.257 images/s.

## Chain consecutive transformer linears into one fused XS kernel

```diff
diff --git a/edgestyle_amd/csrc/builder.hip b/edgestyle_amd/csrc/builder.hip
--- a/edgestyle_amd/csrc/builder.hip
+++ b/edgestyle_amd/csrc/builder.hip
@@ -411,6 +411,36 @@
   if (q.geglu || q.has_ln || q.kpad % groups || !xs_shape_fits(q.ksize, q.kpad, q.cin, q.ctail, q.cout, false)) return false;
   if (q.M < (q.kpad == 320 ? 8192 : 32768)) return false;
   return !(q.ngroups > 1 && (q.ngroups > 4 || !groups_tile_256(q) || !q.groups_agree));
+}
+int xs_chain_classes = ES_XS_CHAIN_A | ES_XS_CHAIN_B;
+int launch_chain(const es_launch_query& q1, int gn_groups1, const es_launch_query& q2, const es_launch_knobs& k) {
+  if (!k.xs_enabled || q1.dtype != ES_F16 || q2.dtype != ES_F16 || q1.M != q2.M || q1.ngroups != q2.ngroups) return 0;
+  if (q1.kpad != 320 || q1.cout != 320 || q1.geglu || q1.has_ln || q2.kpad != 320 || !q2.has_ln || q2.has_residual) return 0;
+  es_launch_knobs k0 = k;
+  k0.xs_min_m = 0;
+  if (gn_groups1 > 0) { if (q1.has_residual || !launch_gn_fold(q1, gn_groups1, k)) return 0; }
+  else if (!launch_takes_xs(q1, k0)) return 0;
+  if (!launch_takes_xs(q2, k0)) return 0;
+  for (int g = 0; g < 4 && q1.ngroups > 1; ++g) if (q1.group_n[g] * q1.hw != q2.group_n[g] * q2.hw) return 0;
+  if (k.xs_min_m && q1.M < k.xs_min_m) return 0;
+  const long long wide = std::max<long long>(320, q2.geglu ? q2.cout / 2 : q2.cout) * 2;
+  if ((q1.M + 256) * wide >= 0x7FFFFFFFll) return 0;
+  const int cls = gn_groups1 > 0 ? ES_XS_CHAIN_A : q2.geglu ? ES_XS_CHAIN_C : ES_XS_CHAIN_B;
+  if (!(xs_chain_classes & cls)) return 0;
+  if (q1.M < 4 * (long long)XS_MIN_M && !(xs_chain_classes & ES_XS_CHAIN_SMALL_M)) return 0;
+  return cls;
+}
+void xs_chain_slices(long long M, int cout2, bool geglu2, int32_t* nslices, int32_t* chunks_per_slice) {
+  const int pline = geglu2 ? 2 : 1, lines = cout2 / 64 / pline;
+  const long long rbs = (M + 255) / 256;
+  long long best = 0; int bl = lines;
+  for (int lps = lines; lps >= 1; --lps) {
+    const int ns = cdiv(lines, lps);
+    if (cdiv(lines, ns) != lps) continue;
+    const long long t = ((rbs * ns + XS_TARGET_WGS - 1) / XS_TARGET_WGS) * (9 + lps * pline);
+    if (!best || t < best) { best = t; bl = lps; }
+  }
+  *nslices = cdiv(lines, bl); *chunks_per_slice = bl * pline;
 }
 struct BuildEnv { es_launch_knobs knobs; bool chunk_major; };
 BuildEnv read_build_env() {
@@ -830,6 +860,94 @@
     if (grouped) for (int n : group_n) rows.push_back(n * hw);
     linear_xs(x.view((int)M, 1, 1, x.c), pl, M, out.view((int)M, 1, 1, pl[0]->cout), rows, T(), &gn);
     return out;
+  }
+
+  void linear_xs_chain(const T& x, const PWs& p1, const PWs& p2, long long M, const T& out1, const T& out2, const std::vector<long long>& group_rows,
+                       const T& residual, const GnFront* gn) {
+    const PW *a = p1[0], *b = p2[0];
+    es_xs_chain_desc d;
+    memset(&d, 0, sizeof(d));
+    auto bias_of = [&](const PW* q) -> unsigned long long {
+      if (q->bias) return q->bias;
+      auto it = zero_bias.find(q->rows_padded);
+      if (it != zero_bias.end()) return it->second;
+      return zero_bias[q->rows_padded] = persistent((size_t)q->rows_padded * 4);
+    };
+    d.x = x.ptr(); d.out1 = out1.ptr(); d.out2 = out2.ptr();
+    d.w1 = (const void*)a->w; d.bias1 = (const float*)bias_of(a); d.w2 = (const void*)b->w; d.bias2 = (const float*)bias_of(b);
+    d.M = (int)M; d.K = a->kpad; d.dtype = dt;
+    d.Cout1 = a->cout; d.rows_padded1 = a->rows_padded; d.ldo1 = out1.c;
+    d.Cout2 = b->cout; d.rows_padded2 = b->rows_padded; d.ldo2 = out2.c; d.geglu2 = b->geglu; d.ln_eps = b->ln_eps;
+    es_xs_chain_slices(M, b->cout, b->geglu, &d.nslices, &d.chunks_per_slice);
+    if (residual) d.residual = residual.ptr();
+    if (gn) {
+      d.gn_part = (const float*)gn->part; d.gn_groups = gn->groups; d.gn_nchunk = gn->nchunk; d.gn_hw = gn->hw; d.gn_eps = gn->eps;
+      if (p1.size() > 1) {
+        if (gn->nl.size() != p1.size()) fail("grouped linear_xs_chain: one GroupNorm parameter set per weight group");
+        for (size_t g = 0; g < p1.size(); ++g) { d.gn_gamma_g[g] = (const float*)gn->nl[g].g; d.gn_beta_g[g] = (const float*)gn->nl[g].b; }
+      } else { d.gn_gamma = (const float*)gn->nl[0].g; d.gn_beta = (const float*)gn->nl[0].b; }
+    }
+    if (p1.size() > 1) {
+      if (p2.size() != p1.size()) fail("grouped linear_xs_chain: one weight set per group and stage");
+      d.ngroups = (int)p1.size();
+      long long acc = 0;
+      for (size_t g = 0; g < p1.size(); ++g) {
+        const PW *q1 = p1[g], *q2 = p2[g];
+        if (q1->rows_padded != a->rows_padded || q1->kpad != a->kpad || q1->cout != a->cout || q2->rows_padded != b->rows_padded || q2->kpad != b->kpad ||
+            q2->cout != b->cout || q2->geglu != b->geglu) fail("grouped linear_xs_chain: weight geometry differs between groups");
+        acc += group_rows[g] / 128;
+        d.mt_end[g] = (int)acc;
+        d.w1_g[g] = (const void*)q1->w; d.bias1_g[g] = (const float*)bias_of(q1); d.w2_g[g] = (const void*)q2->w; d.bias2_g[g] = (const float*)bias_of(q2);
+      }
+    }
+    ok(es_linear_xs_chain(&d, nullptr), "es_linear_xs_chain");
+  }
+  es_launch_query consumer_query(const PWs& p2, long long M, const std::vector<int>& rows) const {
+    CA c; c.group_n = rows;
+    return launch_query(p2, M, 1, c, p2[0]->cin, 0, M * p2[0]->cin, false);
+  }
+  bool linear_chain(const T& x, const PWs& p1, const T& residual, const PWs& p2, const std::vector<int>& rows, T* tok, T* y) {
+    const long long M = x.numel() / x.c;
+    if (!x.contig() || !residual || !residual.contig() || residual.numel() != M * p1[0]->cout) return false;
+    CA c; c.group_n = rows; c.residual = residual; c.wide = true;
+    const es_launch_query q1 = launch_query(p1, M, 1, c, x.c, 0, x.numel(), true);
+    const es_launch_query q2 = consumer_query(p2, M, rows);
+    if (!launch_chain(q1, 0, q2, env.knobs)) return false;
+    const int c2 = p2[0]->geglu ? p2[0]->cout / 2 : p2[0]->cout;
+    T o1 = empty(x.n, x.h, x.w, p1[0]->cout), o2 = empty(x.n, x.h, x.w, c2);
+    std::vector<long long> gr(rows.begin(), rows.end());
+    linear_xs_chain(x.view((int)M, 1, 1, x.c), p1, p2, M, o1.view((int)M, 1, 1, o1.c), o2.view((int)M, 1, 1, c2), gr, residual.view((int)M, 1, 1, o1.c), nullptr);
+    *tok = o1; *y = o2;
+    return true;
+  }
+  bool gn_proj_in_chain(const T& x, const std::vector<Norm>& nl, int groups, float eps, const PWs& p1, const PWs& p2, const std::vector<int>& group_n,
+                        T* tok, T* y) {
+    const int N = x.n;
+    const long long hw = x.hw(), M = (long long)N * hw;
+    CA g; g.group_n = group_n;
+    es_launch_query q1 = launch_query(p1, M, hw, g, x.c, 0, x.numel(), false);
+    for (const PW* p : p1)
+      if (p->rows_padded != p1[0]->rows_padded || p->kpad != p1[0]->kpad || p->cout != p1[0]->cout || p->geglu != p1[0]->geglu) q1.groups_agree = 0;
+    std::vector<int> rows;
+    for (int n : group_n) rows.push_back((int)(n * hw));
+    const es_launch_query q2 = consumer_query(p2, M, rows);
+    if (!x.contig() || !launch_chain(q1, groups, q2, env.knobs)) return false;
+    auto key = std::make_pair(N, groups);
+    auto it = gn_partials.find(key);
+    if (it == gn_partials.end()) it = gn_partials.emplace(key, persistent(es_group_norm_partials_bytes(N, groups))).first;
+    es_gn_desc d;
+    memset(&d, 0, sizeof(d));
+    d.x = x.ptr(); d.partials = (float*)it->second;
+    d.N = N; d.HW = (int)hw; d.C1 = x.c; d.C2 = 0; d.groups = groups; d.eps = eps; d.silu = 0; d.dtype = dt; d.stats_only = 1;
+    ok(es_group_norm(&d, nullptr), "es_group_norm");
+    const int c2 = p2[0]->geglu ? p2[0]->cout / 2 : p2[0]->cout;
+    T o1 = empty(N, x.h, x.w, p1[0]->cout), o2 = empty(N, x.h, x.w, c2);
+    GnFront gn;
+    gn.part = it->second; gn.nl = nl; gn.groups = groups; gn.nchunk = es_group_norm_chunks((int)hw); gn.hw = (int)hw; gn.eps = eps;
+    std::vector<long long> gr(rows.begin(), rows.end());
+    linear_xs_chain(x.view((int)M, 1, 1, x.c), p1, p2, M, o1.view((int)M, 1, 1, o1.c), o2.view((int)M, 1, 1, c2), gr, T(), &gn);
+    *tok = o1; *y = o2;
+    return true;
   }
 
   T timestep_embedding(const T& t, int n, int dim) {
@@ -1185,17 +1303,22 @@
     for (int n : counts) rows.push_back(n * H * Wd);
     std::vector<Norm> nl; PWs pin, qkv, o1, q2, o2, ff1, ffo;
     for (auto t : ts) { nl.push_back(t->norm); pin.push_back(t->proj_in); qkv.push_back(t->qkv_ln); o1.push_back(t->o1); q2.push_back(t->q2_ln); o2.push_back(t->o2); ff1.push_back(t->ff1_ln); ffo.push_back(t->ffo); }
-    T tok = B.gn_proj_in(x, nl, t0->groups, 1e-6f, pin, counts).view(Nn, H * Wd, 1, C);
     CA gr; gr.group_n = rows;
-    T q = B.linear(tok, qkv, gr);
+    T tok, q, qq, f;
+    if (B.gn_proj_in_chain(x, nl, t0->groups, 1e-6f, pin, qkv, counts, &tok, &q)) { tok = tok.view(Nn, H * Wd, 1, C); q = q.view(Nn, H * Wd, 1, 3 * C); }
+    else { tok = B.gn_proj_in(x, nl, t0->groups, 1e-6f, pin, counts).view(Nn, H * Wd, 1, C); q = B.linear(tok, qkv, gr); }
     T a = B.attention(q.chan(0, C), q.chan(C, C), q.chan(2 * C, C), t0->heads);
-    CA r1 = gr; r1.residual = tok; r1.wide = true;
-    tok = B.linear(a, o1, r1);
-    T qq = B.linear(tok, q2, gr);
+    if (!B.linear_chain(a, o1, tok, q2, rows, &tok, &qq)) {
+      CA r1 = gr; r1.residual = tok; r1.wide = true;
+      tok = B.linear(a, o1, r1);
+      qq = B.linear(tok, q2, gr);
+    }
     a = B.attention(qq, kv.chan(0, C), kv.chan(C, C), t0->heads);
-    CA r2 = gr; r2.residual = tok; r2.wide = true;
-    tok = B.linear(a, o2, r2);
-    T f = B.linear(tok, ff1, gr);
+    if (!B.linear_chain(a, o2, tok, ff1, rows, &tok, &f)) {
+      CA r2 = gr; r2.residual = tok; r2.wide = true;
+      tok = B.linear(a, o2, r2);
+      f = B.linear(tok, ff1, gr);
+    }
     CA fo; fo.x2 = tok.view(Nn, H, Wd, C); fo.residual = x; fo.group_n = counts; fo.wide = true; fo.gn_groups = t0->groups;
     return B.conv_gemm(f.view(Nn, H, Wd, 4 * C), ffo, fo);
   }
@@ -1224,16 +1347,25 @@
   }
   T transformer(const Transformer& t, const T& x, const T& kv) {
     const int Nn = x.n, H = x.h, Wd = x.w, C = x.c;
-    T tok = B.gn_proj_in(x, std::vector<Norm>{t.norm}, t.groups, 1e-6f, PWs{t.proj_in}).view(Nn, H * Wd, 1, C);
-    T q = B.linear(tok, t.qkv_ln);
+    T tok, q, qq, f;
+    if (B.gn_proj_in_chain(x, std::vector<Norm>{t.norm}, t.groups, 1e-6f, PWs{t.proj_in}, PWs{t.qkv_ln}, {}, &tok, &q)) {
+      tok = tok.view(Nn, H * Wd, 1, C); q = q.view(Nn, H * Wd, 1, 3 * C);
+    } else {
+      tok = B.gn_proj_in(x, std::vector<Norm>{t.norm}, t.groups, 1e-6f, PWs{t.proj_in}).view(Nn, H * Wd, 1, C);
+      q = B.linear(tok, t.qkv_ln);
+    }
     T a = B.attention(q.chan(0, C), q.chan(C, C), q.chan(2 * C, C), t.heads);
-    CA r1; r1.residual = tok; r1.wide = true;
-    tok = B.linear(a, t.o1, r1);
-    T qq = B.linear(tok, t.q2_ln);
+    if (!B.linear_chain(a, PWs{t.o1}, tok, PWs{t.q2_ln}, {}, &tok, &qq)) {
+      CA r1; r1.residual = tok; r1.wide = true;
+      tok = B.linear(a, t.o1, r1);
+      qq = B.linear(tok, t.q2_ln);
+    }
     a = B.attention(qq, kv.chan(0, C), kv.chan(C, C), t.heads);
-    CA r2; r2.residual = tok; r2.wide = true;
-    tok = B.linear(a, t.o2, r2);
-    T f = B.linear(tok, t.ff1_ln);
+    if (!B.linear_chain(a, PWs{t.o2}, tok, PWs{t.ff1_ln}, {}, &tok, &f)) {
+      CA r2; r2.residual = tok; r2.wide = true;
+      tok = B.linear(a, t.o2, r2);
+      f = B.linear(tok, t.ff1_ln);
+    }
     CA fo; fo.x2 = tok.view(Nn, H, Wd, C); fo.residual = x; fo.wide = true; fo.gn_groups = t.groups;
     return B.conv_gemm(f.view(Nn, H, Wd, 4 * C), t.ffo, fo);
   }
@@ -1542,6 +1674,13 @@
   if (!launch_choose(*q, *k, out)) { es_set_error("es_launch_choose: rows_padded fits no N tile"); return -1; }
   return 0;
 }
+extern "C" int es_launch_chain(const es_launch_query* q1, int gn_groups1, const es_launch_query* q2, const es_launch_knobs* k) {
+  return q1 && q2 && k ? launch_chain(*q1, gn_groups1, *q2, *k) : 0;
+}
+extern "C" void es_xs_chain_slices(long long M, int cout2, int geglu2, int32_t* nslices, int32_t* chunks_per_slice) {
+  xs_chain_slices(M, cout2, geglu2 != 0, nslices, chunks_per_slice);
+}
+extern "C" int es_linear_xs_chain_set_classes(int mask) { const int prev = xs_chain_classes; xs_chain_classes = mask; return prev; }
 extern "C" int es_launch_route(const es_launch_query* q, const es_launch_knobs* k) { return q && k && launch_takes_xs(*q, *k) ? ES_ROUTE_LINEAR_XS : ES_ROUTE_CONV_GEMM; }
 extern "C" int es_launch_gn_fold(const es_launch_query* q, int groups, const es_launch_knobs* k) { return q && k && launch_gn_fold(*q, groups, *k); }
 extern "C" int es_launch_gn_handover(long long hw, int c, int groups, const es_launch_knobs* k) { return k && gn_handover(hw, c, groups, *k); }
diff --git a/edgestyle_amd/csrc/elementwise.hip b/edgestyle_amd/csrc/elementwise.hip
--- a/edgestyle_amd/csrc/elementwise.hip
+++ b/edgestyle_amd/csrc/elementwise.hip
@@ -358,6 +358,7 @@
     case 3: return sizeof(es_fusion_desc);
     case 4: return sizeof(es_ln_desc);
     case 5: return sizeof(es_xs_desc);
+    case 6: return sizeof(es_xs_chain_desc);
     default: return 0;
   }
 }
diff --git a/edgestyle_amd/csrc/linear_xs_chain.hip b/edgestyle_amd/csrc/linear_xs_chain.hip
--- /dev/null
+++ b/edgestyle_amd/csrc/linear_xs_chain.hip
@@ -0,0 +1,388 @@
+#ifndef ES_WT_STORES
+#define ES_WT_STORES 1
+#endif
+#include "common.h"
+#include "../../include/edgestyle_hip.h"
+#include "plan.h"
+
+namespace {
+
+typedef __attribute__((address_space(3))) void* lptr_t;
+
+constexpr int XS_ROWS = 256;
+constexpr int XS_STAGES = 3;
+constexpr int XS_STAGE_W = 40960;
+constexpr int XS_STAGE = XS_STAGE_W + 256;
+constexpr int XS_OROW = 144;
+constexpr int XS_LDS = XS_STAGES * XS_STAGE + 8 * 32 * XS_OROW;
+
+template <int N> ES_DEVICE void wait_vm() { asm volatile("s_waitcnt vmcnt(%0)" ::"n"(N) : "memory"); }
+
+#ifndef XSC_WPF
+#define XSC_WPF 2
+#endif
+template <bool GN, bool RES, bool GEGLU2>
+__global__ __launch_bounds__(512, 2) void linear_xs_chain_kernel(const es_xs_chain_desc p) {
+  typedef f16 T;
+  constexpr int KC = 10, K = 320, NF = 4, CH = 64, SUB = CH * 128, PPS = CH / 8, S1 = K / CH;
+  constexpr int OUTB2 = GEGLU2 ? CH : CH * 2, P2 = 128 / OUTB2;
+  constexpr int NDMA = 6, ST = 4, RS = RES ? 4 : 0, WPF = XSC_WPF;
+  static_assert(!(GN && RES), "GroupNorm in front: no residual");
+  extern __shared__ __attribute__((aligned(16))) char smem[];
+
+  const int tid = threadIdx.x;
+  const int lane = tid & 63;
+  const int wave = __builtin_amdgcn_readfirstlane(tid >> 6);
+  const int frow = lane & 15, fq = lane >> 4;
+  const int slice = blockIdx.x % p.nslices, rb = blockIdx.x / p.nslices;
+  if (p.prof && tid == 0) atomicMin(p.prof, (unsigned long long)__builtin_amdgcn_s_memrealtime());
+
+  const int total2 = p.Cout2 / CH;
+  const int c0 = slice * p.chunks_per_slice;
+  int c1 = c0 + p.chunks_per_slice;
+  c1 = c1 < total2 ? c1 : total2;
+  const int nt = S1 + (c1 - c0);
+
+  int grp = 0;
+  if (p.ngroups > 1) {
+    const int t128 = rb * (XS_ROWS / 128);
+    grp = (t128 >= p.mt_end[0]) + (t128 >= p.mt_end[1]) + (t128 >= p.mt_end[2]);
+  }
+  const bool grouped = p.ngroups > 1;
+  const auto rW1 = __builtin_amdgcn_make_buffer_rsrc((void*)(grouped ? p.w1_g[grp] : p.w1), (short)0, (int)((size_t)p.rows_padded1 * K * 2), 0x00020000);
+  const auto rB1 = __builtin_amdgcn_make_buffer_rsrc((void*)(grouped ? p.bias1_g[grp] : p.bias1), (short)0, (int)((size_t)p.rows_padded1 * 4), 0x00020000);
+  const auto rW2 = __builtin_amdgcn_make_buffer_rsrc((void*)(grouped ? p.w2_g[grp] : p.w2), (short)0, (int)((size_t)p.rows_padded2 * K * 2), 0x00020000);
+  const auto rB2 = __builtin_amdgcn_make_buffer_rsrc((void*)(grouped ? p.bias2_g[grp] : p.bias2), (short)0, (int)((size_t)p.rows_padded2 * 4), 0x00020000);
+  const auto rX = __builtin_amdgcn_make_buffer_rsrc((void*)p.x, (short)0, (int)((size_t)p.M * K * 2), 0x00020000);
+
+  const int lrow = lane >> 3;
+  const int kc8 = (lane & 7) ^ lrow;
+  const unsigned wvoff = (unsigned)((lrow * K + kc8 * 8) * 2);
+  auto ring = [&](int t) __attribute__((always_inline)) { int stg = t % XS_STAGES; asm volatile("" : "+s"(stg)); return stg; };
+  auto issue = [&](int t) __attribute__((always_inline)) {
+    char* sb = smem + ring(t) * XS_STAGE;
+    const bool s1 = t < S1;
+    const int n0 = (s1 ? t : c0 + t - S1) * CH;
+    const auto rW = s1 ? rW1 : rW2;
+    const auto rB = s1 ? rB1 : rB2;
+#pragma unroll
+    for (int i = 0; i < 5; ++i) {
+      const int piece = wave * 5 + i;
+      const int st = piece / PPS, g = piece - st * PPS;
+      __builtin_amdgcn_raw_ptr_buffer_load_lds(rW, (lptr_t)(sb + st * SUB + g * 1024), 16, (int)wvoff, ((n0 + g * 8) * K + st * 64) * 2, 0, 0);
+    }
+    __builtin_amdgcn_raw_ptr_buffer_load_lds(rB, (lptr_t)(sb + XS_STAGE_W), 4, lane * 4, n0 * 4, 0, 0);
+  };
+
+  char* ostage = smem + XS_STAGES * XS_STAGE + wave * (32 * XS_OROW);
+  const int r0 = rb * XS_ROWS + wave * 32;
+  f16x8 xr[2][KC], xr2[2][KC];
+#pragma unroll
+  for (int rf = 0; rf < 2; ++rf)
+#pragma unroll
+    for (int kc = 0; kc < KC; ++kc) {
+      const int row = r0 + rf * 16 + frow;
+      const unsigned off = row < p.M ? (unsigned)(((size_t)row * K + kc * 32 + fq * 8) * 2) : 0xFFFFFF00u;
+      xr[rf][kc] = as_vec8<T>(__builtin_bit_cast(u32x4, __builtin_amdgcn_raw_buffer_load_b128(rX, (int)off, 0, 0)));
+    }
+  if constexpr (GN) {
+    float* gst = (float*)(smem + XS_STAGES * XS_STAGE);
+    const int n = (int)(((long long)rb * XS_ROWS) / p.gn_hw);
+    const int G = p.gn_groups, cpg = K / G;
+    const float inv_cnt = 1.0f / ((float)cpg * (float)p.gn_hw);
+    for (int g0 = 0; g0 < G; g0 += 32) {
+      const int g = g0 + (tid >> 4), l = tid & 15;
+      float s = 0.f, ss = 0.f;
+      if (g < G)
+        for (int ch = l; ch < p.gn_nchunk; ch += 16) {
+          const float* q = p.gn_part + (((size_t)n * p.gn_nchunk + ch) * G + g) * 2;
+          s += q[0]; ss += q[1];
+        }
+      s += dpp_mov<0xB1>(s); ss += dpp_mov<0xB1>(ss);
+      s += dpp_mov<0x4E>(s); ss += dpp_mov<0x4E>(ss);
+      s += dpp_mov<0x141>(s); ss += dpp_mov<0x141>(ss);
+      s += dpp_mov<0x140>(s); ss += dpp_mov<0x140>(ss);
+      if (g < G && l == 0) {
+        const float mean = s * inv_cnt;
+        float var = ss * inv_cnt - mean * mean;
+        var = var < 0.f ? 0.f : var;
+        const float rstd = rsqrtf(var + p.gn_eps);
+        gst[g * 2] = rstd;
+        gst[g * 2 + 1] = -mean * rstd;
+      }
+    }
+    asm volatile("s_waitcnt lgkmcnt(0)" ::: "memory");
+    __builtin_amdgcn_s_barrier();
+  }
+  issue(0);
+  issue(1);
+  if constexpr (GN) {
+    const float* gsel = grouped ? p.gn_gamma_g[grp] : p.gn_gamma;
+    const float* bsel2 = grouped ? p.gn_beta_g[grp] : p.gn_beta;
+    const float* gst = (const float*)(smem + XS_STAGES * XS_STAGE);
+    const int cpg = K / p.gn_groups;
+    const unsigned inv = ((1u << 20) + (unsigned)cpg - 1u) / (unsigned)cpg;
+#pragma unroll
+    for (int kc = 0; kc < KC; ++kc) {
+      const int cb = kc * 32 + fq * 8;
+      const f32x4 g0v = *(const f32x4*)(gsel + cb), g1v = *(const f32x4*)(gsel + cb + 4);
+      const f32x4 b0v = *(const f32x4*)(bsel2 + cb), b1v = *(const f32x4*)(bsel2 + cb + 4);
+#pragma unroll
+      for (int e = 0; e < 8; ++e) {
+        const int g = (int)(((unsigned)(cb + e) * inv) >> 20);
+        const float gam = e < 4 ? g0v[e & 3] : g1v[e & 3], bet = e < 4 ? b0v[e & 3] : b1v[e & 3];
+        const float a = gst[g * 2] * gam, b = __builtin_fmaf(gst[g * 2 + 1], gam, bet);
+#pragma unroll
+        for (int rf = 0; rf < 2; ++rf) xr[rf][kc][e] = from_f32<T>(__builtin_fmaf(to_f32(xr[rf][kc][e]), a, b));
+      }
+      asm volatile("" : "+v"(xr[0][kc]), "+v"(xr[1][kc]));
+    }
+  }
+
+  const auto rO1 = __builtin_amdgcn_make_buffer_rsrc(p.out1, (short)0, (int)((size_t)p.M * p.ldo1 * 2), 0x00020000);
+  const auto rO2 = __builtin_amdgcn_make_buffer_rsrc(p.out2, (short)0, (int)((size_t)p.M * p.ldo2 * 2), 0x00020000);
+  const auto rR = __builtin_amdgcn_make_buffer_rsrc((void*)(RES ? p.residual : p.out1), (short)0, (int)((size_t)p.M * p.ldo1 * 2), 0x00020000);
+  const bool store1 = slice == 0;
+  const bool late = wave >= 4;
+
+  auto load_res = [&](int t, u32x4 (&rr)[4]) __attribute__((always_inline)) {
+    if constexpr (RES) {
+#pragma unroll
+      for (int i = 0; i < 4; ++i) {
+        const int row = i * 8 + (lane >> 3), col = lane & 7;
+        const unsigned off = (unsigned)(((size_t)(r0 + row) * p.ldo1 + t * 64 + col * 8) * 2);
+        rr[i] = __builtin_bit_cast(u32x4, __builtin_amdgcn_raw_buffer_load_b128(rR, (int)off, 0, 0));
+      }
+    }
+  };
+
+  auto compute = [&](int t, const f16x8 (&X)[2][KC], f32x4 (&acc)[NF][2], f32x4 (&bias)[NF], const int nf0, const int nfn) __attribute__((always_inline)) {
+    const char* sb = smem + ring(t) * XS_STAGE;
+    f16x8 wf[WPF + 1][NF];
+#pragma unroll
+    for (int a = 0; a < WPF; ++a)
+#pragma unroll
+      for (int nf = 0; nf < nfn; ++nf) {
+        const int st = a >> 1, h = a & 1, row = (nf0 + nf) * 16 + frow;
+        wf[a][nf] = as_vec8<T>(*(const u32x4*)(sb + st * SUB + row * 128 + (((4 * h + fq) ^ (row & 7)) << 4)));
+      }
+#pragma unroll
+    for (int nf = 0; nf < nfn; ++nf) bias[nf] = *(const f32x4*)(sb + XS_STAGE_W + ((nf0 + nf) * 16 + fq * 4) * 4);
+#pragma unroll
+    for (int kc = 0; kc < KC; ++kc) {
+#pragma unroll
+      for (int nf = 0; nf < nfn; ++nf) {
+        if (kc + WPF < KC) {
+          const int k2 = kc + WPF, st = k2 >> 1, h = k2 & 1, row = (nf0 + nf) * 16 + frow;
+          wf[k2 % (WPF + 1)][nf] = as_vec8<T>(*(const u32x4*)(sb + st * SUB + row * 128 + (((4 * h + fq) ^ (row & 7)) << 4)));
+        }
+        __builtin_amdgcn_sched_barrier(0);
+        acc[nf][0] = mfma16(wf[kc % (WPF + 1)][nf], X[0][kc], kc == 0 ? bias[nf] : acc[nf][0]);
+        acc[nf][1] = mfma16(wf[kc % (WPF + 1)][nf], X[1][kc], kc == 0 ? bias[nf] : acc[nf][1]);
+        __builtin_amdgcn_sched_barrier(0);
+      }
+    }
+  };
+  auto stage_half = [&](const f32x4 (&acc)[NF][2], const int nf0) __attribute__((always_inline)) {
+#pragma unroll
+    for (int nf = 0; nf < 2; ++nf)
+#pragma unroll
+      for (int rf = 0; rf < 2; ++rf) {
+        f16x4 pk;
+#pragma unroll
+        for (int r = 0; r < 4; ++r) pk[r] = from_f32<T>(acc[nf][rf][r]);
+        *(f16x4*)(ostage + (rf * 16 + frow) * XS_OROW + ((nf0 + nf) * 16 + fq * 4) * 2) = pk;
+      }
+  };
+
+  float lns[2] = {0.f, 0.f}, lnss[2] = {0.f, 0.f};
+  auto epilogue1 = [&](int t, const u32x4 (&rr)[4]) __attribute__((always_inline)) {
+    if constexpr (RES) { if (t + 2 < nt) wait_vm<NDMA>(); else wait_vm<0>(); }
+#pragma unroll
+    for (int i = 0; i < 4; ++i) {
+      const int row = i * 8 + (lane >> 3), col = lane & 7;
+      u32x4 v = *(const u32x4*)(ostage + row * XS_OROW + col * 16);
+      if constexpr (RES) {
+        auto a = as_vec8<T>(v);
+        const auto b = as_vec8<T>(rr[i]);
+#pragma unroll
+        for (int e = 0; e < 8; ++e) a[e] = from_f32<T>(to_f32(a[e]) + to_f32(b[e]));
+        v = __builtin_bit_cast(u32x4, a);
+        *(u32x4*)(ostage + row * XS_OROW + col * 16) = v;
+      }
+      const unsigned off = store1 ? (unsigned)(((size_t)(r0 + row) * p.ldo1 + t * 64 + col * 8) * 2) : 0xFFFFFF00u;
+      __builtin_amdgcn_raw_buffer_store_b128(v, rO1, (int)off, 0, ES_WT_STORES ? 16 : 0);
+    }
+#pragma unroll
+    for (int rf = 0; rf < 2; ++rf)
+#pragma unroll
+      for (int h = 0; h < 2; ++h) {
+        xr2[rf][2 * t + h] = as_vec8<T>(*(const u32x4*)(ostage + (rf * 16 + frow) * XS_OROW + (h * 32 + fq * 8) * 2));
+#pragma unroll
+        for (int e = 0; e < 8; ++e) { const float v = to_f32(xr2[rf][2 * t + h][e]); lns[rf] += v; lnss[rf] = __builtin_fmaf(v, v, lnss[rf]); }
+        asm volatile("" : "+v"(xr2[rf][2 * t + h]), "+v"(lns[rf]), "+v"(lnss[rf]));
+      }
+  };
+  auto normalise = [&]() __attribute__((always_inline)) {
+#pragma unroll
+    for (int rf = 0; rf < 2; ++rf) {
+      const float s = xor32_sum(xor16_sum(lns[rf]));
+      const float ss = xor32_sum(xor16_sum(lnss[rf]));
+      const float mean = s * (1.0f / (float)K);
+      float var = ss * (1.0f / (float)K) - mean * mean;
+      var = var < 0.f ? 0.f : var;
+      const float rstd = rsqrtf(var + p.ln_eps);
+      const float shift = -mean * rstd;
+#pragma unroll
+      for (int kc = 0; kc < KC; ++kc) {
+#pragma unroll
+        for (int e = 0; e < 8; ++e) xr2[rf][kc][e] = from_f32<T>(__builtin_fmaf(to_f32(xr2[rf][kc][e]), rstd, shift));
+        asm volatile("" : "+v"(xr2[rf][kc]));
+      }
+    }
+  };
+  auto epilogue2 = [&](int u, const f32x4 (&acc)[NF][2]) __attribute__((always_inline)) {
+    const int sub = u % P2;
+#pragma unroll
+    for (int nf = 0; nf < NF; nf += (GEGLU2 ? 2 : 1))
+#pragma unroll
+      for (int rf = 0; rf < 2; ++rf) {
+        f16x4 pk;
+#pragma unroll
+        for (int r = 0; r < 4; ++r) {
+          if constexpr (GEGLU2) pk[r] = from_f32<T>(acc[nf][rf][r] * gelu_f(acc[nf + 1][rf][r]));
+          else pk[r] = from_f32<T>(acc[nf][rf][r]);
+        }
+        const int chan = (GEGLU2 ? nf / 2 : nf) * 16 + fq * 4;
+        *(f16x4*)(ostage + (rf * 16 + frow) * XS_OROW + sub * OUTB2 + chan * 2) = pk;
+      }
+    if (sub == P2 - 1) {
+      const int line = (c0 + u) / P2;
+#pragma unroll
+      for (int i = 0; i < 4; ++i) {
+        const int row = i * 8 + (lane >> 3), col = lane & 7;
+        const u32x4 v = *(const u32x4*)(ostage + row * XS_OROW + col * 16);
+        const unsigned off = (unsigned)(((size_t)(r0 + row) * p.ldo2 + line * 64 + col * 8) * 2);
+        __builtin_amdgcn_raw_buffer_store_b128(v, rO2, (int)off, 0, ES_WT_STORES ? 16 : 0);
+      }
+    }
+  };
+  auto stores_of = [&](int t) { return t < 0 ? 0 : (t < S1 || ((t - S1) % P2) == P2 - 1) ? ST : 0; };
+
+  f32x4 acc[NF][2], bia[NF];
+  u32x4 rr[4];
+  wait_vm<NDMA>();
+  if (late) __builtin_amdgcn_s_barrier();
+#pragma unroll
+  for (int t = 0; t < S1; ++t) {
+    __builtin_amdgcn_s_barrier();
+    load_res(t, rr);
+    compute(t, xr, acc, bia, 0, 2);
+    stage_half(acc, 0);
+    compute(t, xr, acc, bia, 2, 2);
+    stage_half(acc, 2);
+    if (late) {
+      if (t == 0) wait_vm<RS>(); else wait_vm<ST + RS>();
+    }
+    __builtin_amdgcn_s_barrier();
+    if (t + 2 < nt) issue(t + 2);
+    epilogue1(t, rr);
+    if (t == S1 - 1) normalise();
+    if (!late) {
+      if (t + 2 < nt) wait_vm<NDMA + ST>(); else wait_vm<ST>();
+    }
+  }
+  for (int t = S1; t < nt; ++t) {
+    __builtin_amdgcn_s_barrier();
+    compute(t, xr2, acc, bia, 0, NF);
+    if (late && t + 1 < nt) {
+      if (stores_of(t - 1)) wait_vm<ST>(); else wait_vm<0>();
+    }
+    if (!late || t + 1 < nt) __builtin_amdgcn_s_barrier();
+    if (t + 2 < nt) issue(t + 2);
+    epilogue2(t - S1, acc);
+    if (!late && t + 1 < nt) {
+      if (t + 2 < nt) { if (stores_of(t)) wait_vm<NDMA + ST>(); else wait_vm<NDMA>(); }
+      else { if (stores_of(t)) wait_vm<ST>(); else wait_vm<0>(); }
+    }
+  }
+  if (p.prof && tid == 0) atomicMax(p.prof + 1, (unsigned long long)__builtin_amdgcn_s_memrealtime());
+}
+
+int xs_chain_launches = 0;
+
+template <bool GN, bool RES, bool GEGLU2>
+int launch_chain(const es_xs_chain_desc& d, hipStream_t st) {
+  const int rbs = (d.M + XS_ROWS - 1) / XS_ROWS;
+  auto kfn = linear_xs_chain_kernel<GN, RES, GEGLU2>;
+  static bool attr_set = false;
+  if (!attr_set) {
+    (void)hipFuncSetAttribute((const void*)kfn, hipFuncAttributeMaxDynamicSharedMemorySize, XS_LDS);
+    attr_set = true;
+  }
+  ++xs_chain_launches;
+  hipLaunchKernelGGL(kfn, dim3(rbs * d.nslices), dim3(512), XS_LDS, st, d);
+  return hipGetLastError() == hipSuccess ? 0 : -2;
+}
+
+}
+
+extern "C" void es_set_error(const char* msg);
+
+extern unsigned long long es_operand_limit_v;
+
+extern "C" int es_linear_xs_chain_launches(void) { return xs_chain_launches; }
+
+extern "C" int es_linear_xs_chain(const es_xs_chain_desc* d, void* stream) {
+  const bool grouped = d->ngroups > 1;
+  if (!d->x || !d->out1 || !d->out2 || (!grouped && (!d->w1 || !d->bias1 || !d->w2 || !d->bias2))) {
+    es_set_error("es_linear_xs_chain: null pointer (biases are required: pass zeros)"); return -1; }
+  if (d->K != 320) { es_set_error("es_linear_xs_chain: K must be 320"); return -1; }
+  if (d->dtype != ES_F16) { es_set_error("es_linear_xs_chain: fp16 only (bf16 carries the two-word residual stream: two es_linear_xs / es_conv_gemm calls)"); return -1; }
+  if (d->Cout1 != 320 || d->rows_padded1 < 320) { es_set_error("es_linear_xs_chain: stage 1 must be a 320 -> 320 projection"); return -1; }
+  const int P2 = d->geglu2 ? 2 : 1;
+  if (d->M < 1 || d->Cout2 < 64 || d->Cout2 % (64 * P2) || d->rows_padded2 < d->Cout2) {
+    es_set_error("es_linear_xs_chain: Cout2 must be a multiple of the 128-byte output line (64 stored channels)"); return -1; }
+  const int total2 = d->Cout2 / 64;
+  if (d->nslices < 1 || d->chunks_per_slice < P2 || d->chunks_per_slice % P2 ||
+      (long long)d->nslices * d->chunks_per_slice < total2 || (long long)(d->nslices - 1) * d->chunks_per_slice >= total2) {
+    es_set_error("es_linear_xs_chain: slices must cover Cout2 in whole output lines, none empty"); return -1; }
+  const int cstore2 = d->geglu2 ? d->Cout2 / 2 : d->Cout2;
+  if (d->ldo1 < 320 || d->ldo1 % 8 || d->ldo2 < cstore2 || d->ldo2 % 8) { es_set_error("es_linear_xs_chain: bad output pitch"); return -1; }
+  if ((size_t)d->rows_padded2 * 320 * 2 >= 0x7FFFFFFFull || (size_t)d->rows_padded1 * 320 * 2 >= 0x7FFFFFFFull) {
+    es_set_error("es_linear_xs_chain: weights larger than 2 GiB (32-bit buffer offsets)"); return -1; }
+  const size_t wide = (size_t)(d->ldo1 > d->ldo2 ? d->ldo1 : d->ldo2) * 2;
+  if ((size_t)d->M * 320 * 2 >= es_operand_limit_v || ((size_t)d->M + 256) * wide >= es_operand_limit_v) {
+    es_set_error("es_linear_xs_chain: operands beyond 32-bit buffer offsets (run the pair as two es_linear_xs calls)"); return -1; }
+  if (d->ngroups > 4) { es_set_error("es_linear_xs_chain: at most 4 groups"); return -1; }
+  if (d->gn_part) {
+    if (d->residual) { es_set_error("es_linear_xs_chain: GroupNorm in front (gn_part) takes no residual"); return -1; }
+    if (d->gn_groups < 1 || d->gn_groups > 32 || 320 % d->gn_groups || d->gn_hw < 256 || d->gn_hw % 256 || d->M % d->gn_hw || d->gn_nchunk < 1 || d->gn_nchunk > 64) {
+      es_set_error("es_linear_xs_chain: gn_part needs 1..32 groups dividing K, samples of a whole number of 256-row blocks covering M, 1..64 chunks"); return -1; }
+    if (!grouped && (!d->gn_gamma || !d->gn_beta)) { es_set_error("es_linear_xs_chain: gn_part without gn_gamma / gn_beta"); return -1; }
+    for (int g = 0; g < d->ngroups && grouped; ++g) {
+      if (!d->gn_gamma_g[g] || !d->gn_beta_g[g]) { es_set_error("es_linear_xs_chain: gn_part without gn_gamma_g / gn_beta_g for every group"); return -1; }
+      if (((long long)d->mt_end[g] * 128) % d->gn_hw) { es_set_error("es_linear_xs_chain: gn_part needs weight groups of whole samples (mt_end * 128 a multiple of gn_hw)"); return -1; }
+    }
+  }
+  if (d->residual && d->nslices > 1 && d->residual == d->out1) {
+    es_set_error("es_linear_xs_chain: with several slices the residual must not alias out1 (every slice reads it, one writes)"); return -1; }
+  es_xs_chain_desc dd = *d;
+  if (grouped) {
+    const int tm = (d->M + 127) / 128;
+    for (int g = 0; g < d->ngroups; ++g)
+      if (!d->w1_g[g] || !d->bias1_g[g] || !d->w2_g[g] || !d->bias2_g[g] || d->mt_end[g] <= (g ? d->mt_end[g - 1] : 0) ||
+          (g + 1 < d->ngroups && (d->mt_end[g] & 1))) {
+        es_set_error("es_linear_xs_chain: groups must be non-empty runs of whole 256-row blocks (the last may be ragged)"); return -1; }
+    if (d->mt_end[d->ngroups - 1] != tm) { es_set_error("es_linear_xs_chain: groups must cover M"); return -1; }
+  }
+  for (int g = grouped ? dd.ngroups : 0; g < 4; ++g) dd.mt_end[g] = 0x7FFFFFFF;
+  ES_PLAN_RECORD(ES_OP_LINEAR_XS_CHAIN, d, sizeof(*d));
+  hipStream_t st = (hipStream_t)stream;
+  int rc;
+  if (dd.gn_part) rc = dd.geglu2 ? launch_chain<true, false, true>(dd, st) : launch_chain<true, false, false>(dd, st);
+  else if (dd.residual) rc = dd.geglu2 ? launch_chain<false, true, true>(dd, st) : launch_chain<false, true, false>(dd, st);
+  else rc = dd.geglu2 ? launch_chain<false, false, true>(dd, st) : launch_chain<false, false, false>(dd, st);
+  if (rc) es_set_error("es_linear_xs_chain: launch failed");
+  return rc;
+}
diff --git a/edgestyle_amd/csrc/plan.h b/edgestyle_amd/csrc/plan.h
--- a/edgestyle_amd/csrc/plan.h
+++ b/edgestyle_amd/csrc/plan.h
@@ -6,7 +6,7 @@
   ES_OP_CONV_GEMM = 1, ES_OP_LINEAR_XS, ES_OP_ATTENTION, ES_OP_GROUP_NORM, ES_OP_LAYER_NORM, ES_OP_LAYER_NORM_GROUPED,
   ES_OP_FUSION_BLOCK, ES_OP_FUSION_BLOCKS, ES_OP_TIMESTEP_EMBEDDING, ES_OP_CFG_DDIM, ES_OP_CFG_UNIPC, ES_OP_NCHW_TO_NHWC,
   ES_OP_NHWC_TO_NCHW, ES_OP_ADD, ES_OP_VAE_SAMPLE, ES_OP_INCR, ES_OP_GATHER_ROW, ES_OP_MEMCPY, ES_OP_MEMCPY2D,
-  ES_OP_FILL_F32, ES_OP_LATENTS_TO_INPUT,
+  ES_OP_FILL_F32, ES_OP_LATENTS_TO_INPUT, ES_OP_LINEAR_XS_CHAIN,
 };
 
 struct es_op_layer_norm { const void* x; void* out; const float* gamma; const float* beta; int M, C; float eps; int dtype; };
diff --git a/edgestyle_amd/csrc/plan.hip b/edgestyle_amd/csrc/plan.hip
--- a/edgestyle_amd/csrc/plan.hip
+++ b/edgestyle_amd/csrc/plan.hip
@@ -35,6 +35,7 @@
   switch (op.kind) {
     case ES_OP_CONV_GEMM: return es_conv_gemm((const es_gemm_desc*)a, s);
     case ES_OP_LINEAR_XS: return es_linear_xs((const es_xs_desc*)a, s);
+    case ES_OP_LINEAR_XS_CHAIN: return es_linear_xs_chain((const es_xs_chain_desc*)a, s);
     case ES_OP_ATTENTION: return es_attention((const es_attn_desc*)a, s);
     case ES_OP_GROUP_NORM: return es_group_norm((const es_gn_desc*)a, s);
     case ES_OP_LAYER_NORM: { auto* r = (const es_op_layer_norm*)a; return es_layer_norm(r->x, r->out, r->gamma, r->beta, r->M, r->C, r->eps, r->dtype, s); }
@@ -130,6 +131,12 @@
         F_IN(es_xs_desc, x), F_OUT(es_xs_desc, out), F_IN(es_xs_desc, w), F_IN(es_xs_desc, bias), F_IN4(es_xs_desc, w_g),
         F_IN4(es_xs_desc, bias_g), F_OUT(es_xs_desc, prof), F_IN(es_xs_desc, residual), F_IN(es_xs_desc, gn_part), F_IN(es_xs_desc, gn_gamma),
         F_IN(es_xs_desc, gn_beta), F_IN4(es_xs_desc, gn_gamma_g), F_IN4(es_xs_desc, gn_beta_g)}; return f; }
+    case ES_OP_LINEAR_XS_CHAIN: { static const std::vector<PtrField> f = {
+        F_IN(es_xs_chain_desc, x), F_OUT(es_xs_chain_desc, out1), F_IN(es_xs_chain_desc, w1), F_IN(es_xs_chain_desc, bias1), F_IN4(es_xs_chain_desc, w1_g),
+        F_IN4(es_xs_chain_desc, bias1_g), F_IN(es_xs_chain_desc, residual), F_IN(es_xs_chain_desc, gn_part), F_IN(es_xs_chain_desc, gn_gamma),
+        F_IN(es_xs_chain_desc, gn_beta), F_IN4(es_xs_chain_desc, gn_gamma_g), F_IN4(es_xs_chain_desc, gn_beta_g), F_OUT(es_xs_chain_desc, out2),
+        F_IN(es_xs_chain_desc, w2), F_IN(es_xs_chain_desc, bias2), F_IN4(es_xs_chain_desc, w2_g), F_IN4(es_xs_chain_desc, bias2_g),
+        F_OUT(es_xs_chain_desc, prof)}; return f; }
     case ES_OP_ATTENTION: { static const std::vector<PtrField> f = {
         F_IN(es_attn_desc, q), F_IN(es_attn_desc, k), F_IN(es_attn_desc, v), F_OUT(es_attn_desc, o)}; return f; }
     case ES_OP_GROUP_NORM: { static const std::vector<PtrField> f = {
diff --git a/edgestyle_amd/engine.py b/edgestyle_amd/engine.py
--- a/edgestyle_amd/engine.py
+++ b/edgestyle_amd/engine.py
@@ -132,15 +132,27 @@
 
     def __call__(self, x, kv):
         N, H, W, C = x.shape
-        tok = ops.gn_proj_in(x, self.norm[0], self.norm[1], self.groups, 1e-6, self.proj_in).reshape(N, H * W, C)
         fold = self.ln_fold
-        qkv = ops.linear(tok, self.qkv_ln) if fold else ops.linear(ops.layer_norm(tok, *self.ln1), self.qkv)
+        pair = ops.gn_proj_in_chain(x, self.norm[0], self.norm[1], self.groups, 1e-6, self.proj_in, self.qkv_ln) if fold else None
+        if pair is not None:
+            tok, qkv = pair[0].reshape(N, H * W, C), pair[1].reshape(N, H * W, 3 * C)
+        else:
+            tok = ops.gn_proj_in(x, self.norm[0], self.norm[1], self.groups, 1e-6, self.proj_in).reshape(N, H * W, C)
+            qkv = ops.linear(tok, self.qkv_ln) if fold else ops.linear(ops.layer_norm(tok, *self.ln1), self.qkv)
         a = ops.attention(qkv[:, :, :C], qkv[:, :, C:2 * C], qkv[:, :, 2 * C:], self.heads)
-        tok = ops.linear(a, self.o1, residual=tok, wide=True)
-        q = ops.linear(tok, self.q2_ln) if fold else ops.linear(ops.layer_norm(tok, *self.ln2), self.q2)
+        pair = ops.linear_chain(a, self.o1, tok, self.q2_ln) if fold else None
+        if pair is not None:
+            tok, q = pair
+        else:
+            tok = ops.linear(a, self.o1, residual=tok, wide=True)
+            q = ops.linear(tok, self.q2_ln) if fold else ops.linear(ops.layer_norm(tok, *self.ln2), self.q2)
         a = ops.attention(q, kv[:, :, :C], kv[:, :, C:], self.heads)
-        tok = ops.linear(a, self.o2, residual=tok, wide=True)
-        f = ops.linear(tok, self.ff1_ln) if (fold and self.ff1_ln is not None) else ops.linear(ops.layer_norm(tok, *self.ln3), self.ff1)
+        pair = ops.linear_chain(a, self.o2, tok, self.ff1_ln) if (fold and self.ff1_ln is not None) else None
+        if pair is not None:
+            tok, f = pair
+        else:
+            tok = ops.linear(a, self.o2, residual=tok, wide=True)
+            f = ops.linear(tok, self.ff1_ln) if (fold and self.ff1_ln is not None) else ops.linear(ops.layer_norm(tok, *self.ln3), self.ff1)
         if self.ffo is not None:
             return ops.conv_gemm(f.reshape(N, H, W, 4 * C), self.ffo, x2=tok.reshape(N, H, W, C), residual=x, wide=True, gn_groups=self.groups)
         tok = ops.linear(f, self.ff2, residual=tok, wide=True)
@@ -460,21 +472,37 @@
         t0 = ts[0]
         N, H, W, C = x.shape
         rows = [n * H * W for n in c]
-        tok = ops.gn_proj_in(x, [t.norm[0] for t in ts], [t.norm[1] for t in ts], t0.groups, 1e-6, [t.proj_in for t in ts], group_n=c).reshape(N, H * W, C)
         fold = all(t.ln_fold for t in ts)
+        fold3 = all(t.ln_fold and t.ff1_ln is not None for t in ts)
+        pair = ops.gn_proj_in_chain(x, [t.norm[0] for t in ts], [t.norm[1] for t in ts], t0.groups, 1e-6, [t.proj_in for t in ts],
+                                    [t.qkv_ln for t in ts], group_n=c) if fold else None
+        qkv = None
+        if pair is not None:
+            tok, qkv = pair[0].reshape(N, H * W, C), pair[1].reshape(N, H * W, 3 * C)
+        else:
+            tok = ops.gn_proj_in(x, [t.norm[0] for t in ts], [t.norm[1] for t in ts], t0.groups, 1e-6, [t.proj_in for t in ts], group_n=c).reshape(N, H * W, C)
 
         def ln_linear(k, plain, folded):
             if fold and folded is not None:
                 return ops.linear(tok, [getattr(t, folded) for t in ts], group_n=rows)
             n = ops.layer_norm(tok, [getattr(t, k)[0] for t in ts], [getattr(t, k)[1] for t in ts], group_rows=rows)
             return ops.linear(n, [getattr(t, plain) for t in ts], group_n=rows)
-        qkv = ln_linear("ln1", "qkv", "qkv_ln")
+        if qkv is None:
+            qkv = ln_linear("ln1", "qkv", "qkv_ln")
         a = ops.attention(qkv[:, :, :C], qkv[:, :, C:2 * C], qkv[:, :, 2 * C:], t0.heads)
-        tok = ops.linear(a, [t.o1 for t in ts], residual=tok, group_n=rows, wide=True)
-        q = ln_linear("ln2", "q2", "q2_ln")
+        pair = ops.linear_chain(a, [t.o1 for t in ts], tok, [t.q2_ln for t in ts], group_n=rows) if fold else None
+        if pair is not None:
+            tok, q = pair
+        else:
+            tok = ops.linear(a, [t.o1 for t in ts], residual=tok, group_n=rows, wide=True)
+            q = ln_linear("ln2", "q2", "q2_ln")
         a = ops.attention(q, kv[:, :, :C], kv[:, :, C:], t0.heads)
-        tok = ops.linear(a, [t.o2 for t in ts], residual=tok, group_n=rows, wide=True)
-        f = ln_linear("ln3", "ff1", "ff1_ln" if all(t.ln_fold and t.ff1_ln is not None for t in ts) else None)
+        pair = ops.linear_chain(a, [t.o2 for t in ts], tok, [t.ff1_ln for t in ts], group_n=rows) if fold3 else None
+        if pair is not None:
+            tok, f = pair
+        else:
+            tok = ops.linear(a, [t.o2 for t in ts], residual=tok, group_n=rows, wide=True)
+            f = ln_linear("ln3", "ff1", "ff1_ln" if fold3 else None)
         if all(t.ffo is not None for t in ts):
             return ops.conv_gemm(f.reshape(N, H, W, 4 * C), [t.ffo for t in ts], x2=tok.reshape(N, H, W, C), residual=x, group_n=c, wide=True,
                                  gn_groups=t0.groups)
diff --git a/edgestyle_amd/lib.py b/edgestyle_amd/lib.py
--- a/edgestyle_amd/lib.py
+++ b/edgestyle_amd/lib.py
@@ -44,6 +44,23 @@
     ]
 
 
+class XsChainDesc(C.Structure):
+    _fields_ = [
+        ("x", C.c_void_p), ("out1", C.c_void_p), ("w1", C.c_void_p), ("bias1", C.c_void_p),
+        ("w1_g", C.c_void_p * 4), ("bias1_g", C.c_void_p * 4), ("residual", C.c_void_p),
+        ("gn_part", C.c_void_p), ("gn_gamma", C.c_void_p), ("gn_beta", C.c_void_p), ("gn_gamma_g", C.c_void_p * 4), ("gn_beta_g", C.c_void_p * 4),
+        ("out2", C.c_void_p), ("w2", C.c_void_p), ("bias2", C.c_void_p), ("w2_g", C.c_void_p * 4), ("bias2_g", C.c_void_p * 4),
+        ("prof", C.c_void_p),
+        ("mt_end", C.c_int32 * 4), ("ngroups", C.c_int32),
+        ("M", C.c_int32), ("K", C.c_int32), ("dtype", C.c_int32),
+        ("Cout1", C.c_int32), ("rows_padded1", C.c_int32), ("ldo1", C.c_int32),
+        ("Cout2", C.c_int32), ("rows_padded2", C.c_int32), ("ldo2", C.c_int32), ("geglu2", C.c_int32),
+        ("ln_eps", C.c_float),
+        ("nslices", C.c_int32), ("chunks_per_slice", C.c_int32),
+        ("gn_groups", C.c_int32), ("gn_nchunk", C.c_int32), ("gn_hw", C.c_int32), ("gn_eps", C.c_float),
+    ]
+
+
 class CtxGeometry(C.Structure):
     _fields_ = [("B", C.c_int32), ("cfg", C.c_int32), ("h", C.c_int32), ("w", C.c_int32),
                 ("latent_channels", C.c_int32), ("latent_pad", C.c_int32), ("n_conds", C.c_int32),
@@ -58,6 +75,8 @@
 BUF_HIST0, BUF_COUNT = 30, 33
 SCHED_DDIM, SCHED_UNIPC = 0, 1
 OP_CONV_GEMM, OP_LINEAR_XS, OP_ATTENTION = 1, 2, 3
+OP_LINEAR_XS_CHAIN = 22
+XS_CHAIN_A, XS_CHAIN_B, XS_CHAIN_C, XS_CHAIN_SMALL_M = 1, 2, 4, 8
 
 
 class AttnDesc(C.Structure):
@@ -182,6 +201,11 @@
     "es_conv_gemm": (C.c_int, [C.POINTER(GemmDesc), _P]),
     "es_conv_gemm_workspace_bytes": (C.c_size_t, [C.POINTER(GemmDesc)]),
     "es_linear_xs": (C.c_int, [C.POINTER(XsDesc), _P]),
+    "es_linear_xs_chain": (C.c_int, [C.POINTER(XsChainDesc), _P]),
+    "es_linear_xs_chain_set_classes": (C.c_int, [_I]),
+    "es_linear_xs_chain_launches": (C.c_int, []),
+    "es_launch_chain": (C.c_int, [C.POINTER(LaunchQuery), _I, C.POINTER(LaunchQuery), C.POINTER(LaunchKnobs)]),
+    "es_xs_chain_slices": (None, [C.c_longlong, _I, _I, C.POINTER(C.c_int32), C.POINTER(C.c_int32)]),
     "es_linear_xs_set_pp": (C.c_int, [_I]),
     "es_linear_xs_last_form": (C.c_int, []),
     "es_attention": (C.c_int, [C.POINTER(AttnDesc), _P]),
@@ -305,7 +329,7 @@
         fn.argtypes = args
     if lib.es_abi_version() != ABI_VERSION:
         raise EdgeStyleHipError("libedgestyle_hip.so ABI version mismatch")
-    for i, st in enumerate((GemmDesc, AttnDesc, GnDesc, FusionDesc, LnDesc, XsDesc)):
+    for i, st in enumerate((GemmDesc, AttnDesc, GnDesc, FusionDesc, LnDesc, XsDesc, XsChainDesc)):
         if lib.es_sizeof_desc(i) != C.sizeof(st):
             raise EdgeStyleHipError(f"descriptor layout mismatch for {st.__name__}: C {lib.es_sizeof_desc(i)} "
                                     f"vs ctypes {C.sizeof(st)}")
diff --git a/edgestyle_amd/ops.py b/edgestyle_amd/ops.py
--- a/edgestyle_amd/ops.py
+++ b/edgestyle_amd/ops.py
@@ -59,9 +59,9 @@
     def replay_gemms(self, only_ksize: int = 0):
         lib = L.load()
         for d in self.descs:
-            if only_ksize and (isinstance(d, L.XsDesc) or int(d.ksize) != only_ksize):
+            if only_ksize and (isinstance(d, (L.XsDesc, L.XsChainDesc)) or int(d.ksize) != only_ksize):
                 continue
-            fn = lib.es_linear_xs if isinstance(d, L.XsDesc) else lib.es_conv_gemm
+            fn = lib.es_linear_xs if isinstance(d, L.XsDesc) else lib.es_linear_xs_chain if isinstance(d, L.XsChainDesc) else lib.es_conv_gemm
             L.check(fn(C.byref(d), _stream()), "GEMM replay")
 
     def results(self, first: int = 0):
@@ -461,6 +461,132 @@
         PROFILE.descs.append(dd)
     L.check(L.load().es_linear_xs(C.byref(d), _stream()), "es_linear_xs")
     return out
+
+
+def linear_xs_chain(x: torch.Tensor, pw1, pw2, M: int, out1: torch.Tensor, out2: torch.Tensor, group_rows=None,
+                    residual: Optional[torch.Tensor] = None, gn: Optional[dict] = None, slices=None):
+    def bad(msg):
+        return L.EdgeStyleHipError("linear_xs_chain: " + msg)
+    pws1 = pws2 = None
+    if isinstance(pw1, (list, tuple)):
+        if not isinstance(pw2, (list, tuple)) or len(pw2) != len(pw1):
+            raise bad("one weight set per group and stage")
+        if len(pw1) > 1:
+            pws1, pws2 = list(pw1), list(pw2)
+        pw1, pw2 = pw1[0], pw2[0]
+    c2 = pw2.cout // 2 if pw2.geglu else pw2.cout
+    if x.dtype not in (torch.float16, torch.bfloat16):
+        raise bad(f"x must be fp16, not {x.dtype}")
+    if pw2.ln_colsum is None:
+        raise bad("stage 2 must be LayerNorm-folded weights (ops.pack_weight_ln)")
+    if M < 1 or x.dim() != 2 or tuple(x.shape) != (M, pw1.kpad) or not x.is_contiguous():
+        raise bad(f"x must be a contiguous [M, K] = [{M}, {pw1.kpad}] (got shape {tuple(x.shape)}, strides {x.stride()})")
+    for name, t, c in (("out1", out1, pw1.cout), ("out2", out2, c2), ("residual", residual, pw1.cout)):
+        if t is None:
+            continue
+        if t.dtype != x.dtype or t.device != x.device:
+            raise bad(f"{name} is {t.dtype} on {t.device}, x is {x.dtype} on {x.device}")
+        if t.dim() != 2 or tuple(t.shape) != (M, c) or t.stride(1) != 1:
+            raise bad(f"{name} must be [M, {c}] with innermost stride 1, not {tuple(t.shape)} / {t.stride()}")
+        if t.device.type != "meta" and t.data_ptr() % 16:
+            raise bad(f"{name} must start at a multiple of 16 bytes (16-byte vector accesses)")
+    if x.device.type != "meta" and x.data_ptr() % 16:
+        raise bad("x must start at a multiple of 16 bytes (16-byte vector loads)")
+    ldo1 = out1.stride(0) if M > 1 else pw1.cout
+    ldo2 = out2.stride(0) if M > 1 else c2
+    if ldo1 < pw1.cout or ldo1 % 8 or ldo2 < c2 or ldo2 % 8:
+        raise bad(f"row pitches {ldo1} / {ldo2} must be multiples of 8 elements and at least the widths {pw1.cout} / {c2}")
+    if residual is not None and M > 1 and residual.stride(0) != ldo1:
+        raise bad(f"residual: row pitch {residual.stride(0)} differs from out1's {ldo1} (the kernel reads it with out1's)")
+    if pws1 is not None:
+        if group_rows is None or len(group_rows) != len(pws1) or sum(group_rows) != M or any(n < 1 for n in group_rows):
+            raise bad(f"group_rows {None if group_rows is None else list(group_rows)} must hold one run of rows per weight set and sum to M = {M}")
+        if any(n % 256 for n in list(group_rows)[:-1]):
+            raise bad(f"group_rows {list(group_rows)}: every run but the last must be whole 256-row blocks")
+    lib = L.load()
+    d = L.XsChainDesc()
+    d.x, d.out1, d.out2 = x.data_ptr(), out1.data_ptr(), out2.data_ptr()
+
+    def bias_of(q):
+        if q.bias is not None:
+            return q.bias.data_ptr()
+        key = (x.device, q.rows_padded)
+        z = _zero_bias.get(key)
+        if z is None:
+            z = _zero_bias[key] = torch.zeros(q.rows_padded, dtype=torch.float32, device=x.device)
+        return z.data_ptr()
+    d.w1, d.bias1, d.w2, d.bias2 = pw1.w.data_ptr(), bias_of(pw1), pw2.w.data_ptr(), bias_of(pw2)
+    d.M, d.K, d.dtype = M, pw1.kpad, _dt(x)
+    d.Cout1, d.rows_padded1, d.ldo1 = pw1.cout, pw1.rows_padded, ldo1
+    d.Cout2, d.rows_padded2, d.ldo2, d.geglu2, d.ln_eps = pw2.cout, pw2.rows_padded, ldo2, int(pw2.geglu), pw2.ln_eps
+    if slices is not None:
+        d.nslices, d.chunks_per_slice = slices
+    else:
+        ns, cps = C.c_int32(), C.c_int32()
+        lib.es_xs_chain_slices(M, pw2.cout, int(pw2.geglu), C.byref(ns), C.byref(cps))
+        d.nslices, d.chunks_per_slice = ns.value, cps.value
+    d.residual = residual.data_ptr() if residual is not None else None
+    if gn is not None:
+        d.gn_part, d.gn_groups, d.gn_nchunk, d.gn_hw, d.gn_eps = gn["part"].data_ptr(), gn["groups"], gn["nchunk"], gn["hw"], gn["eps"]
+        gam, bet = gn["gamma"], gn["beta"]
+        if pws1 is not None:
+            if len(gam) != len(pws1) or len(bet) != len(pws1):
+                raise bad("one GroupNorm parameter set per weight group")
+            for g in range(len(pws1)):
+                d.gn_gamma_g[g], d.gn_beta_g[g] = gam[g].data_ptr(), bet[g].data_ptr()
+        else:
+            if isinstance(gam, (list, tuple)):
+                gam, bet = gam[0], bet[0]
+            d.gn_gamma, d.gn_beta = gam.data_ptr(), bet.data_ptr()
+    if pws1 is not None:
+        d.ngroups = len(pws1)
+        acc = 0
+        for g, (q1, q2, n) in enumerate(zip(pws1, pws2, group_rows)):
+            if (q1.rows_padded, q1.kpad, q1.cout) != (pw1.rows_padded, pw1.kpad, pw1.cout) or \
+                    (q2.rows_padded, q2.kpad, q2.cout, q2.geglu) != (pw2.rows_padded, pw2.kpad, pw2.cout, pw2.geglu):
+                raise bad("weight geometry differs between groups")
+            acc += n
+            d.mt_end[g] = (acc + 127) // 128
+            d.w1_g[g], d.bias1_g[g], d.w2_g[g], d.bias2_g[g] = q1.w.data_ptr(), bias_of(q1), q2.w.data_ptr(), bias_of(q2)
+    if PROFILE is not None:
+        K = pw1.kpad
+        nbytes = _algorithmic_bytes(x, None, pw1, pws1, out1, residual) + out2.numel() * out2.element_size() + \
+            sum(q.w.numel() * q.w.element_size() for q in (pws2 if pws2 is not None else [pw2]))
+        d.prof = PROFILE.next((2.0 * M * (pw1.cout + pw2.cout) * K, 1, (M, pw1.cout + pw2.cout, K, 1, 1, 0),
+                               dict(N=M, H=1, W=1, C1=K, C2=0, cout=pw1.cout + pw2.cout, k=1, stride=1, pad=0, upsample=False,
+                                    geglu=pw2.geglu, splitk=1, Hout=1, Wout=1, residual=residual is not None, temb=False, bn=0, stages=3,
+                                    group_n=list(group_rows) if pws1 is not None else None, ctail=0, kernel="linear_xs_chain",
+                                    algorithmic_bytes=nbytes)))
+        dd = L.XsChainDesc()
+        C.memmove(C.byref(dd), C.byref(d), C.sizeof(L.XsChainDesc))
+        dd.prof = None
+        PROFILE.descs.append(dd)
+    L.check(lib.es_linear_xs_chain(C.byref(d), _stream()), "es_linear_xs_chain")
+    return out1, out2
+
+
+def _consumer_query(M: int, pw2, pws2, rows, x):
+    return launch_query(M, 1, pw2, pws2, rows, src_numel=M * pw2.cin, C1=pw2.cin, dtype=_dt(x))
+
+
+def linear_chain(x: torch.Tensor, pw1, residual: torch.Tensor, pw2, group_n: Optional[Sequence[int]] = None):
+    shp = x.shape
+    M = x.numel() // shp[-1]
+    l1, l2 = (list(pw1), list(pw2)) if isinstance(pw1, (list, tuple)) else ([pw1], [pw2])
+    p1, p2 = l1[0], l2[0]
+    pws1, pws2 = (l1, l2) if len(l1) > 1 else (None, None)
+    if not x.is_contiguous() or residual is None or not residual.is_contiguous() or residual.numel() != M * p1.cout or x.dtype not in _DT:
+        return None
+    q1 = launch_query(M, 1, p1, pws1, group_n, src_numel=x.numel(), C1=shp[-1], has_residual=1, wide=1, dtype=_dt(x))
+    q2 = _consumer_query(M, p2, pws2, group_n, x)
+    if not L.load().es_launch_chain(C.byref(q1), 0, C.byref(q2), C.byref(launch_knobs())):
+        return None
+    c2 = p2.cout // 2 if p2.geglu else p2.cout
+    tok = torch.empty((*shp[:-1], p1.cout), dtype=x.dtype, device=x.device)
+    y = torch.empty((*shp[:-1], c2), dtype=x.dtype, device=x.device)
+    linear_xs_chain(x.reshape(M, shp[-1]), l1, l2, M, tok.reshape(M, p1.cout), y.reshape(M, c2),
+                    None if pws1 is None else list(group_n), residual=residual.reshape(M, p1.cout))
+    return tok, y
 
 
 WIDE_STREAM = _os.environ.get("ES_WIDE_STREAM", "auto")
@@ -836,6 +962,37 @@
     return out
 
 
+def gn_proj_in_chain(x: torch.Tensor, gamma, beta, groups: int, eps: float, pw, pw2, group_n: Optional[Sequence[int]] = None):
+    N, H, W, Cc, _ = _gn_operands("gn_proj_in", x, None, groups)
+    l1, l2 = (list(pw), list(pw2)) if isinstance(pw, (list, tuple)) else ([pw], [pw2])
+    pws, pws2 = (l1, l2) if len(l1) > 1 else (None, None)
+    p0, p2 = l1[0], l2[0]
+    gl, bl = _norm_params("gn_proj_in", gamma, beta, Cc, x, nsets=None if pws is None else len(pws))
+    M, hw = N * H * W, H * W
+    if x.dtype not in _DT:
+        return None
+    q1 = launch_query(M, hw, p0, pws, group_n)
+    q1.dtype = _dt(x)
+    if pws is not None:
+        q1.groups_agree = all((p.rows_padded, p.kpad, p.cout, p.geglu, p.ln_colsum is None) == (p0.rows_padded, p0.kpad, p0.cout, p0.geglu, True) for p in pws)
+    rows = None if group_n is None else [n * hw for n in group_n]
+    q2 = _consumer_query(M, p2, pws2, rows, x)
+    if not L.load().es_launch_chain(C.byref(q1), groups, C.byref(q2), C.byref(launch_knobs())):
+        return None
+    part = _gn_partials_for("gn_proj_in", x, N, groups)
+    d = L.GnDesc()
+    d.x, d.partials = x.data_ptr(), part.data_ptr()
+    d.N, d.HW, d.C1, d.C2, d.groups = N, hw, Cc, 0, groups
+    d.eps, d.silu, d.dtype, d.stats_only = eps, 0, _dt(x), 1
+    L.check(L.load().es_group_norm(C.byref(d), _stream()), "es_group_norm")
+    c2 = p2.cout // 2 if p2.geglu else p2.cout
+    tok = torch.empty((N, H, W, p0.cout), dtype=x.dtype, device=x.device)
+    y = torch.empty((N, H, W, c2), dtype=x.dtype, device=x.device)
+    linear_xs_chain(x.reshape(M, Cc), l1, l2, M, tok.reshape(M, p0.cout), y.reshape(M, c2), rows,
+                    gn=dict(part=part, gamma=gl, beta=bl, groups=groups, nchunk=L.load().es_group_norm_chunks(hw), hw=hw, eps=eps))
+    return tok, y
+
+
 def layer_norm(x: torch.Tensor, gamma, beta, eps: float = 1e-5, group_rows: Optional[Sequence[int]] = None,
                out: Optional[torch.Tensor] = None) -> torch.Tensor:
     if x.dim() < 1 or x.dtype not in (torch.float16, torch.bfloat16):
diff --git a/include/edgestyle_hip.h b/include/edgestyle_hip.h
--- a/include/edgestyle_hip.h
+++ b/include/edgestyle_hip.h
@@ -86,6 +86,34 @@
 enum { ES_XS_FORM_KC_MASK = 0xFF, ES_XS_FORM_GEGLU = 0x100, ES_XS_FORM_LN = 0x200, ES_XS_FORM_RES = 0x400, ES_XS_FORM_PP = 0x800,
        ES_XS_FORM_GN = 0x1000 };
 int es_linear_xs_last_form(void);
+
+typedef struct {
+  const void* x; void* out1;
+  const void* w1; const float* bias1;
+  const void* w1_g[4]; const float* bias1_g[4];
+  const void* residual;
+  const float* gn_part;
+  const float* gn_gamma; const float* gn_beta;
+  const float* gn_gamma_g[4]; const float* gn_beta_g[4];
+  void* out2;
+  const void* w2; const float* bias2;
+  const void* w2_g[4]; const float* bias2_g[4];
+  unsigned long long* prof;
+  int32_t mt_end[4];
+  int32_t ngroups;
+  int32_t M, K, dtype;
+  int32_t Cout1, rows_padded1, ldo1;
+  int32_t Cout2, rows_padded2, ldo2, geglu2;
+  float ln_eps;
+  int32_t nslices, chunks_per_slice;
+  int32_t gn_groups, gn_nchunk, gn_hw;
+  float gn_eps;
+} es_xs_chain_desc;
+int es_linear_xs_chain(const es_xs_chain_desc* d, void* stream);
+int es_linear_xs_chain_launches(void);
+enum { ES_XS_CHAIN_A = 1 , ES_XS_CHAIN_B = 2 , ES_XS_CHAIN_C = 4 ,
+       ES_XS_CHAIN_SMALL_M = 8  };
+int es_linear_xs_chain_set_classes(int mask);
 
 typedef struct {
   const void* q; const void* k; const void* v; void* o;
@@ -322,6 +350,8 @@
 int es_launch_gn_fold(const es_launch_query* q, int groups, const es_launch_knobs* k);
 int es_launch_gn_handover(long long hw, int c, int groups, const es_launch_knobs* k);
 int es_launch_wide_stream(int dtype, const es_launch_knobs* k);
+int es_launch_chain(const es_launch_query* q1, int gn_groups1, const es_launch_query* q2, const es_launch_knobs* k);
+void es_xs_chain_slices(long long M, int cout2, int geglu2, int32_t* nslices, int32_t* chunks_per_slice);
 int es_conv_gemm8p_form_ok(int act, int cout, int has_temb, long long out_hw, int has_residual);
 int es_ctx_graph_hazard(void);
 int es_plan_set_dry(int on);
```

New measurement: 2.261 images/s, median of 6. About the same (+0.2%).
